# torn8to/sift-based-OD

Hardware: NVIDIA B200
Metric: query descriptors/sec (kNN2+ratio+Hough+affine), 1M-desc DB (higher is better)
Workload: dtype u8

## Files before the change

include/sod.h:

```cpp
#ifndef SOD_H_
#define SOD_H_

#include <stddef.h>
#include <stdint.h>

#ifdef __cplusplus
extern "C" {
#endif

#define SOD_OK 0
#define SOD_ERR_INVALID_ARGUMENT (-1)
#define SOD_ERR_CUDA (-2)
#define SOD_ERR_UNSUPPORTED (-3)

#define SOD_DESC_DIM 128
#define SOD_TILE_ROWS 128
#define SOD_CQ_TILE_INTS 260

typedef void* sod_stream_t;

int sod_version(void);
const char* sod_last_error(void);
int sod_device_sm_count(void);

#define SOD_STAGE_MATCH 0
#define SOD_STAGE_HOUGH_PREP 1
#define SOD_STAGE_HOUGH_VOTE 2
#define SOD_STAGE_HOUGH_FINISH 3
#define SOD_STAGE_AFFINE 4
#define SOD_STAGE_COUNT 5
int sod_timing_enable(int32_t on);
int32_t sod_timing_read(int32_t stage, float* ms_host, int32_t cap);

int64_t sod_cq_ints(int64_t n_rows);

int sod_pack_u8_from_f32(const float* src, int64_t n_rows, uint8_t* dst, int32_t* nonint_flag,
                         sod_stream_t stream);

size_t sod_db_prepare_workspace_bytes(int64_t n_rows);
int sod_db_prepare(const uint8_t* db, int64_t n_rows, uint8_t* db_sorted, int32_t* cq, void* workspace,
                   size_t workspace_bytes, sod_stream_t stream);

int sod_query_prepare(const uint8_t* q, int64_t n_rows, int32_t* qn, sod_stream_t stream);

size_t sod_match_workspace_bytes(int64_t n_query, int64_t n_db);

int sod_match_top2(const uint8_t* q, const int32_t* qn, int64_t n_query, const uint8_t* db_sorted,
                   const int32_t* cq, int64_t n_db, int32_t db_index_base, int32_t* out_idx,
                   uint32_t* out_d2, void* workspace, size_t workspace_bytes, sod_stream_t stream);

int64_t sod_row_thr_ints(int64_t n_query);
int sod_match_top2_range(const uint8_t* q, const int32_t* qn, int64_t n_query, const uint8_t* db_sorted,
                         const int32_t* cq, int64_t n_db, int32_t db_index_base, int64_t tile_begin,
                         int64_t tile_end, int32_t* row_thr, int32_t* out_idx, uint32_t* out_d2,
                         void* workspace, size_t workspace_bytes, sod_stream_t stream);

int sod_match_top2_peer(const uint8_t* q, const int32_t* qn, int64_t n_query, const uint8_t* db_sorted,
                        const int32_t* cq, int64_t n_db, int32_t db_index_base, int64_t tile_begin,
                        int64_t tile_end, int32_t* row_thr, int32_t* const* peer_thr_host, int32_t n_peers,
                        int64_t block_rotation, int32_t* out_idx, uint32_t* out_d2, void* workspace,
                        size_t workspace_bytes, sod_stream_t stream);

int sod_top2_merge(const int32_t* parts_idx, const uint32_t* parts_d2, int32_t n_parts,
                   int64_t n_query, int32_t* out_idx, uint32_t* out_d2, float* out_dist,
                   uint8_t* out_pass, double ratio, sod_stream_t stream);

int sod_top2_keys(const int32_t* idx, const uint32_t* d2, int64_t n_query, int64_t n_rows, int64_t* keys,
                  sod_stream_t stream);
int sod_top2_merge_keys(const int64_t* parts, int32_t n_parts, int64_t n_rows, int64_t* out, sod_stream_t stream);
int sod_top2_from_keys(const int64_t* keys, int64_t n_query, int32_t* out_idx, uint32_t* out_d2, float* out_dist,
                       uint8_t* out_pass, double ratio, sod_stream_t stream);

#define SOD_EXCHANGE_MAX_RANKS 16
#define SOD_IPC_HANDLE_BYTES 64
size_t sod_exchange_bytes(int64_t max_query, int32_t world);
int sod_exchange_alloc(size_t bytes, void** buffer_out);
int sod_exchange_free(void* buffer);
int sod_ipc_export(const void* buffer, uint8_t* handle_host);
int sod_ipc_open(const uint8_t* handle_host, void** buffer_out);
int sod_ipc_close(void* buffer);
int sod_top2_exchange_peer(const int32_t* idx, const uint32_t* d2, int64_t n_query, int32_t rank, int32_t world,
                           void* const* peer_buffers_host, int64_t max_query, int32_t* out_idx, uint32_t* out_d2,
                           float* out_dist, uint8_t* out_pass, double ratio, sod_stream_t stream);


int64_t sod_bf16_operand_cols(int32_t split);
int64_t sod_bf16_db_rows(int64_t n_rows);

int sod_bf16_prepare(const float* src, int64_t n_rows, int32_t side, int32_t split, uint16_t* dst,
                     float* norms, int32_t* nonfinite_flag, sod_stream_t stream);

size_t sod_match_bf16_workspace_bytes(int64_t n_query, int64_t n_db);

int sod_match_top2_bf16(const uint16_t* q_op, const float* qn, int64_t n_query, const uint16_t* db_op,
                        const float* dn, int64_t n_db, int32_t split, int32_t db_index_base,
                        int32_t* out_idx, float* out_d2, void* workspace, size_t workspace_bytes,
                        sod_stream_t stream);

int sod_top2_merge_f32(const int32_t* parts_idx, const float* parts_d2, int32_t n_parts,
                       int64_t n_query, int32_t* out_idx, float* out_d2, float* out_dist,
                       uint8_t* out_pass, double ratio, sod_stream_t stream);



typedef struct {
  const float* xy;
  const float* angle;
  const int32_t* octave;
  int64_t n;
} sod_keypoints;

typedef struct {
  sod_keypoints query;
  const int32_t* query_frame;
  const int32_t* frame_wh;
  int32_t n_frames;
  sod_keypoints model;
  const int32_t* model_image;
  const double* image_centroid;
  const double* image_size;
  const int32_t* image_group;
  int32_t n_images;
  int32_t groups_per_frame;
} sod_scene;

#define SOD_SIGMA_LUT_MIN (-24)
#define SOD_SIGMA_LUT_LEN 49
#define SOD_MAX_BINS 15
#define SOD_MAX_CLUSTER_BINS 65536

typedef struct {
  double* pose;
  uint32_t* base_bin;
  uint8_t* near_edge;
  int32_t* counters;
  int32_t* bin_group;
  int32_t* bin_code;
  int32_t* bin_count;
  int32_t* bin_offset;
  int64_t* bin_order;
  double* bin_mean;
  int32_t* members;
  int64_t cap_bins;
  int64_t cap_votes;
} sod_hough_out;

size_t sod_compact_scratch_bytes(int64_t n_query);
int sod_compact_matches(const int32_t* idx, const uint8_t* pass, int64_t n_query, int32_t t_lo,
                        int32_t t_hi, int32_t* match_q, int32_t* match_t, int32_t* n_out,
                        void* scratch, sod_stream_t stream);

int sod_estimate_pose(const sod_scene* scene, const int32_t* match_q, const int32_t* match_t,
                      int64_t n_matches, int32_t bins, const int32_t* sigma_lut, double* pose,
                      uint32_t* base_bin, uint8_t* near_edge, sod_stream_t stream);

int sod_pose_bin_index(const double* pose, int64_t n, int32_t bins, int32_t width, int32_t height,
                       const int32_t* sigma_lut, uint32_t* base_bin, sod_stream_t stream);

size_t sod_hough_workspace_bytes(int64_t n_matches, int64_t n_groups);

int sod_hough_vote(const sod_scene* scene, const int32_t* match_q, const int32_t* match_t,
                   int64_t n_matches, const int32_t* n_matches_dev, int32_t bins,
                   const int32_t* sigma_lut, int32_t detail_min_count, const sod_hough_out* out,
                   void* workspace, size_t workspace_bytes, sod_stream_t stream);

int sod_hough_vote_dims(const sod_scene* scene, const int32_t* match_q, const int32_t* match_t,
                        int64_t n_matches, const int32_t* n_matches_dev, int32_t bins_x, int32_t bins_y,
                        int32_t bins_theta, int32_t bins_sigma, const int32_t* sigma_lut,
                        int32_t detail_min_count, const sod_hough_out* out, void* workspace,
                        size_t workspace_bytes, sod_stream_t stream);

typedef struct {
  int32_t* counters;
  int32_t* valid_bin;
  double* params;
  int32_t* votes;
  int32_t* status;
  uint8_t* member_keep;
  int64_t cap_valid;
  int64_t cap_votes;
} sod_affine_out;

int sod_affine_verify(const sod_scene* scene, const int32_t* match_q, const int32_t* match_t,
                      const sod_hough_out* hough, int32_t bins, int32_t vote_threshold,
                      int32_t affine_threshold, double factor_x, double factor_y, int32_t max_passes,
                      const sod_affine_out* out, sod_stream_t stream);

int sod_valid_bin_records(const sod_hough_out* hough, const sod_affine_out* affine, int32_t* out_group,
                          int32_t* out_code, int64_t* out_order, double* out_mean, sod_stream_t stream);

int sod_affine_residual_keep(const float* model_xy, const float* query_xy, int64_t n,
                             const double* params, double x_ref, double y_ref, uint8_t* keep,
                             sod_stream_t stream);


int sod_pose_adjacency(const double* cx, const double* cy, const double* reach_x, const double* reach_y,
                       const int32_t* segment, int64_t n, uint32_t* adj, int32_t* label,
                       sod_stream_t stream);

int sod_angle_adjacency(const double* angle, const int32_t* segment, int64_t n, double max_degrees,
                        uint32_t* adj, int32_t* label, sod_stream_t stream);


#define SOD_SIFT_MAX_OCTAVES 16
#define SOD_SIFT_MAX_CAP (1 << 24)

typedef struct {
  float* xy;
  float* size;
  float* angle;
  float* response;
  int32_t* octave;
  uint8_t* des;
  int32_t* counters;
  int64_t cap;
} sod_sift_out;

size_t sod_sift_workspace_bytes(int32_t width, int32_t height, int64_t max_keypoints);

int sod_sift_extract(const uint8_t* gray, int32_t width, int32_t height, int64_t pitch, const sod_sift_out* out,
                     void* workspace, size_t workspace_bytes, sod_stream_t stream);

int sod_sift_describe(const uint8_t* gray, int32_t width, int32_t height, int64_t pitch, const float* xy,
                      const float* size, const float* angle, const int32_t* octave, int64_t n, uint8_t* des,
                      int32_t* n_invalid, void* workspace, size_t workspace_bytes, sod_stream_t stream);

int64_t sod_sift_level_offset(int32_t width, int32_t height, int32_t octave, int32_t level, int32_t* wh_host);

#ifdef __cplusplus
}
#endif
#endif
```

sift-based-od_b200/csrc/sod_capi.cu:

```cuda
#include <cstring>

#include "sod_common.cuh"

namespace sod {

namespace {
thread_local char g_err[512] = {0};
}

void set_error(const char* fmt, ...) {
  va_list ap;
  va_start(ap, fmt);
  vsnprintf(g_err, sizeof(g_err), fmt, ap);
  va_end(ap);
}

namespace {
constexpr int kTimerRing = 128;
struct StageTimers {
  bool on = false;
  cudaEvent_t ev[SOD_STAGE_COUNT][kTimerRing][2] = {};
  int head[SOD_STAGE_COUNT] = {};
  bool open[SOD_STAGE_COUNT] = {};
};
thread_local StageTimers g_timers;
}

void stage_begin(int stage, cudaStream_t st) {
  StageTimers& t = g_timers;
  if (!t.on || stage < 0 || stage >= SOD_STAGE_COUNT || t.head[stage] >= kTimerRing) return;
  cudaEvent_t& e = t.ev[stage][t.head[stage]][0];
  if (!e && cudaEventCreate(&e) != cudaSuccess) return;
  t.open[stage] = cudaEventRecord(e, st) == cudaSuccess;
}

void stage_end(int stage, cudaStream_t st) {
  StageTimers& t = g_timers;
  if (!t.on || stage < 0 || stage >= SOD_STAGE_COUNT || !t.open[stage]) return;
  t.open[stage] = false;
  cudaEvent_t& e = t.ev[stage][t.head[stage]][1];
  if (!e && cudaEventCreate(&e) != cudaSuccess) return;
  if (cudaEventRecord(e, st) == cudaSuccess) ++t.head[stage];
}

int device_sm_count() {
  int dev = 0, sms = 0;
  if (cudaGetDevice(&dev) != cudaSuccess ||
      cudaDeviceGetAttribute(&sms, cudaDevAttrMultiProcessorCount, dev) != cudaSuccess) {
    set_error("cannot query the current CUDA device: %s", cudaGetErrorString(cudaGetLastError()));
    return -1;
  }
  return sms;
}

}

extern "C" {

int sod_version(void) { return 2000; }

const char* sod_last_error(void) { return sod::g_err; }

int sod_device_sm_count(void) { return sod::device_sm_count(); }

int sod_timing_enable(int32_t on) {
  sod::g_timers.on = on != 0;
  for (int s = 0; s < SOD_STAGE_COUNT; ++s) {
    sod::g_timers.head[s] = 0;
    sod::g_timers.open[s] = false;
  }
  return SOD_OK;
}

int32_t sod_timing_read(int32_t stage, float* ms_host, int32_t cap) {
  sod::StageTimers& t = sod::g_timers;
  if (stage < 0 || stage >= SOD_STAGE_COUNT || (cap > 0 && !ms_host)) {
    sod::set_error("sod_timing_read: bad stage or null buffer");
    return SOD_ERR_INVALID_ARGUMENT;
  }
  const int n = t.head[stage];
  int out = 0;
  for (int i = 0; i < n; ++i) {
    float ms = 0.f;
    if (cudaEventSynchronize(t.ev[stage][i][1]) != cudaSuccess ||
        cudaEventElapsedTime(&ms, t.ev[stage][i][0], t.ev[stage][i][1]) != cudaSuccess) {
      sod::set_error("sod_timing_read: %s", cudaGetErrorString(cudaGetLastError()));
      t.head[stage] = 0;
      return SOD_ERR_CUDA;
    }
    if (out < cap) ms_host[out++] = ms;
  }
  t.head[stage] = 0;
  return out;
}

}
```

sift-based-od_b200/csrc/sod_match.cu:

```cuda
#include <climits>
#include <cub/device/device_radix_sort.cuh>

#include "sod_common.cuh"
#include "sod_ptx.cuh"
#include "sod_tma.cuh"
#include "sod_top2.cuh"

namespace sod {
namespace {

constexpr int kTileM = 128;
constexpr int kQTiles = 4;
constexpr int kBlockQ = kTileM * kQTiles;
constexpr int kAbiBlockQ = 256;
constexpr int kTileN = SOD_TILE_ROWS;
constexpr int kTileBytes = kTileN * SOD_DESC_DIM;
constexpr int kChunk = 32;
constexpr int kCqTile = SOD_CQ_TILE_INTS;
constexpr int kCqPerm = kTileN + 4;
constexpr int kCqTileBytes = kCqTile * 4;
constexpr int kNoKey = 0x7FFFFF;
constexpr int kEpiWarps = 4 * kQTiles;
constexpr int kIssuers = 2;
constexpr int kThreads = (4 + kEpiWarps) * 32;
constexpr int kTmemCols = 512;
constexpr int kRegsLight = 56;
constexpr int kRegsEpilogue = 104;
constexpr int kRegsLaunch = 65536 / kThreads / 8 * 8;
static_assert(128 * kRegsLight + kEpiWarps * 32 * kRegsEpilogue <= kThreads * kRegsLaunch,
              "setmaxnreg budget exceeds the CTA's register pool");

static_assert(kQTiles * kTileN == kTmemCols, "one 128-column accumulator slot per query tile fills TMEM");

constexpr int kStages = 8;
constexpr int kBStageBytes = kTileBytes / 2;
constexpr int kCqSlots = 16;
constexpr int kOffA = 0;
constexpr int kOffB = kOffA + 2 * kQTiles * kTileBytes;
constexpr int kOffCq = kOffB + kStages * kBStageBytes;
constexpr int kOffBar = kOffCq + kCqSlots * kCqTileBytes;
constexpr int kNumBars = 2 * kStages + 4 + 2 * kQTiles + kCqSlots;
constexpr int kOffTmemPtr = kOffBar + kNumBars * 8;
constexpr int kSmemBytes = kOffTmemPtr + 16 + 1024;
static_assert(kCqSlots >= kStages + 2 && (kCqSlots & (kCqSlots - 1)) == 0, "cq ring too shallow");
static_assert(kSmemBytes <= 227 * 1024, "shared memory exceeds the 227 KB a block may use");

struct MatchArgs {
  const int32_t* qn;
  const int32_t* cq;
  uint32_t* part_d2;
  int32_t* part_idx;
  int32_t* row_thr;
  int nq;
  int thr_rows;
  int n_tiles;
  int tile_begin;
  int n_qunits;
  int n_seg;
  int idx_base;
  int n_peers;
  int unit_rot;
  int32_t* peer_thr[SOD_EXCHANGE_MAX_RANKS];
};

__device__ __forceinline__ int imax3(int a, int b, int c) { return max(max(a, b), c); }
struct Top2 {
  long long k1, k2;
  int d2;
  __device__ __forceinline__ void offer(int d, int i) {
    const long long key = (static_cast<long long>(d) << 32) | static_cast<unsigned>(i);
    if (key < k1) {
      k2 = k1;
      k1 = key;
    } else if (key < k2) {
      k2 = key;
    }
    d2 = static_cast<int>(k2 >> 32);
  }
};
constexpr long long kNoKey64 = (static_cast<long long>(kNoKey) << 32) | 0x7FFFFFFF;

__device__ __forceinline__ void top2_chunk(const uint32_t* v, const int4* __restrict__ cp4,
                                           int cmin, const int32_t* __restrict__ perm_s,
                                           int idx_base, Top2& best, int& thr) {
  const int* av = reinterpret_cast<const int*>(v);
  int t[11];
#pragma unroll
  for (int i = 0; i < 10; ++i) t[i] = imax3(av[3 * i], av[3 * i + 1], av[3 * i + 2]);
  t[10] = max(av[30], av[31]);
  const int u0 = imax3(t[0], t[1], t[2]), u1 = imax3(t[3], t[4], t[5]), u2 = imax3(t[6], t[7], t[8]);
  const int u3 = max(t[9], t[10]);
  if (cmin - 2 * max(imax3(u0, u1, u2), u3) > thr) return;
  const int* cp = reinterpret_cast<const int*>(cp4);
  int t1 = INT_MAX, t2 = INT_MAX;
  auto scan = [&](int lo, int hi) {
#pragma unroll
    for (int j = lo; j < hi; ++j) {
      const int key = cp[j] - 512 * av[j];
      const int m = max(t1, key);
      t1 = min(t1, key);
      t2 = min(t2, m);
    }
  };
  if (cmin - 2 * u0 <= thr) scan(0, 9);
  if (cmin - 2 * u1 <= thr) scan(9, 18);
  if (cmin - 2 * u2 <= thr) scan(18, 27);
  if (cmin - 2 * u3 <= thr) scan(27, 32);
  if ((t1 >> 8) > thr) return;
  SOD_DCHECK((t1 & 0xFF) < kTileN && (t2 == INT_MAX || (t2 & 0xFF) < kTileN));
  const int o1 = perm_s[t1 & 0xFF];
  if (o1 >= 0) best.offer(t1 >> 8, idx_base + o1);
  thr = min(thr, best.d2);
  if ((t2 >> 8) <= thr) {
    const int o2 = perm_s[t2 & 0xFF];
    if (o2 >= 0) best.offer(t2 >> 8, idx_base + o2);
    thr = min(thr, best.d2);
  }
}

template <bool kShare, bool kSeeded = false>
__global__ void __launch_bounds__(kThreads, 1)
match_top2_kernel(const __grid_constant__ CUtensorMap tmap_q,
                  const __grid_constant__ CUtensorMap tmap_db, const MatchArgs a) {
  extern __shared__ uint8_t smem_raw[];
  const uint32_t raw_addr = smem_u32(smem_raw);
  const uint32_t base = (raw_addr + 1023u) & ~1023u;
  uint8_t* smem = smem_raw + (base - raw_addr);

  const int warp = threadIdx.x >> 5;
  const int lane = threadIdx.x & 31;
  const uint32_t cta_rank = cluster_ctarank();
  const int unit0 = static_cast<int>(cluster_id_x());
  const int unit_step = static_cast<int>(cluster_count_x());

  const uint32_t bar0 = base + kOffBar;
  auto bar_full = [&](int s) { return bar0 + 8u * s; };
  auto bar_empty = [&](int s) { return bar0 + 8u * (kStages + s); };
  auto bar_afull = [&](int b) { return bar0 + 8u * (2 * kStages + b); };
  auto bar_aempty = [&](int b) { return bar0 + 8u * (2 * kStages + 2 + b); };
  auto bar_tfull = [&](int h) { return bar0 + 8u * (2 * kStages + 4 + h); };
  auto bar_tempty = [&](int h) { return bar0 + 8u * (2 * kStages + 4 + kQTiles + h); };
  auto bar_cqfull = [&](int s) { return bar0 + 8u * (2 * kStages + 4 + 2 * kQTiles + s); };
  volatile uint32_t* tmem_ptr_smem = reinterpret_cast<volatile uint32_t*>(smem + kOffTmemPtr);

  if (warp == 0 && lane == 0) {
    tma_prefetch_desc(&tmap_q);
    tma_prefetch_desc(&tmap_db);
  }
  if (warp == 1 && lane == 0) {
    for (int s = 0; s < kStages; ++s) {
      mbar_init(bar_full(s), 1);
      mbar_init(bar_empty(s), kIssuers);
    }
    for (int b = 0; b < 2; ++b) {
      mbar_init(bar_afull(b), 1);
      mbar_init(bar_aempty(b), kIssuers);
    }
    for (int h = 0; h < kQTiles; ++h) {
      mbar_init(bar_tfull(h), 1);
      mbar_init(bar_tempty(h), 8);
    }
    for (int s = 0; s < kCqSlots; ++s) mbar_init(bar_cqfull(s), 1);
    fence_mbar_init();
  }
  if (warp == 2) {
    tmem_alloc_pair(smem_u32(const_cast<uint32_t*>(tmem_ptr_smem)), kTmemCols);
    tmem_relinquish_pair();
  }
  tc_fence_before();
  cluster_sync_all();
  tc_fence_after();
  const uint32_t tmem_base = *tmem_ptr_smem;

  const int total_units = a.n_qunits * a.n_seg;

  if (warp < 4) {
    if constexpr (kRegsLight < kRegsLaunch)
      setmaxnreg_dec<kRegsLight>();
  if (warp == 0) {
    if (lane == 0) {
      uint32_t step = 0, ucount = 0;
      for (int u = unit0; u < total_units; u += unit_step, ++ucount) {
        const int seg = u / a.n_qunits;
        int qu = u - seg * a.n_qunits + a.unit_rot;
        if (qu >= a.n_qunits) qu -= a.n_qunits;
        const int qb = qu * 2 + static_cast<int>(cta_rank);
        const int t0 = a.tile_begin + static_cast<int>(static_cast<int64_t>(seg) * a.n_tiles / a.n_seg);
        const int t1 = a.tile_begin + static_cast<int>(static_cast<int64_t>(seg + 1) * a.n_tiles / a.n_seg);
        const uint32_t ab = ucount & 1u, aph = (ucount >> 1) & 1u;
        mbar_wait(bar_aempty(ab), aph ^ 1u);
        if (cta_rank == 0) mbar_arrive_expect_tx(bar_afull(ab), 2 * kQTiles * kTileBytes);
        const uint32_t afull_leader = mapa_shared(bar_afull(ab), 0);
        for (int h = 0; h < kQTiles; ++h)
          tma_load_2d_pair(base + kOffA + (ab * kQTiles + h) * kTileBytes, &tmap_q, afull_leader, 0,
                           qb * kBlockQ + h * kTileM);
        for (int t = t0; t < t1; ++t, ++step) {
          const uint32_t s = step % kStages, ph = (step / kStages) & 1u;
          mbar_wait(bar_empty(s), ph ^ 1u);
          if (cta_rank == 0) mbar_arrive_expect_tx(bar_full(s), 2 * kBStageBytes);
          tma_load_2d_pair(base + kOffB + s * kBStageBytes, &tmap_db, mapa_shared(bar_full(s), 0), 0,
                           t * kTileN + static_cast<int>(cta_rank) * (kTileN / 2));
          const uint32_t slot = step % kCqSlots;
          mbar_arrive_expect_tx(bar_cqfull(slot), kCqTileBytes);
          bulk_load_1d(base + kOffCq + slot * kCqTileBytes, a.cq + static_cast<int64_t>(t) * kCqTile,
                       kCqTileBytes, bar_cqfull(slot));
        }
      }
    }
  } else if ((warp == 1 || warp == 3) && cta_rank == 0) {
    const int h0 = warp >> 1;
    constexpr uint32_t idesc = umma_idesc_u8(2 * kTileM, kTileN);
    uint32_t step = 0, ucount = 0;
    for (int u = unit0; u < total_units; u += unit_step, ++ucount) {
      const int seg = u / a.n_qunits;
      const int t0 = a.tile_begin + static_cast<int>(static_cast<int64_t>(seg) * a.n_tiles / a.n_seg);
      const int t1 = a.tile_begin + static_cast<int>(static_cast<int64_t>(seg + 1) * a.n_tiles / a.n_seg);
      const uint32_t ab = ucount & 1u, aph = (ucount >> 1) & 1u;
      mbar_wait(bar_afull(ab), aph);
      const uint32_t a_buf = base + kOffA + ab * (kQTiles * kTileBytes);
      for (int t = t0; t < t1; ++t, ++step) {
        const uint32_t s = step % kStages, ph = (step / kStages) & 1u;
        const uint64_t bdesc = umma_desc_k128(base + kOffB + s * kBStageBytes);
        mbar_wait(bar_full(s), ph);
#pragma unroll
        for (int i = 0; i < kQTiles / kIssuers; ++i) {
          const int h = h0 + kIssuers * i;
          const uint64_t adesc = umma_desc_k128(a_buf + h * kTileBytes);
          if (step >= 1)
            mbar_wait(bar_tempty(h), (step - 1) & 1u);
          tc_fence_after();
          if (elect_one()) {
#pragma unroll
            for (int k = 0; k < SOD_DESC_DIM / 32; ++k)
              umma_i8_pair(tmem_base + h * kTileN, adesc + 2 * k, bdesc + 2 * k, idesc, k > 0);
            umma_commit_pair(bar_tfull(h), 3);
            if (i == kQTiles / kIssuers - 1) umma_commit_pair(bar_empty(s), 3);
          }
          __syncwarp();
        }
      }
      if (elect_one()) umma_commit_pair(bar_aempty(ab), 3);
      __syncwarp();
    }
  }
  } else {
    if constexpr (kRegsEpilogue > kRegsLaunch) setmaxnreg_inc<kRegsEpilogue>();
    const int e = warp - 4;
    const int quad = warp & 3;
    const int h = e >> 2;
    const uint32_t lane_sel = static_cast<uint32_t>(quad * 32) << 16;
    uint32_t tfull_h = bar_tfull(h);
    uint32_t cqfull_0 = bar_cqfull(0);
    uint32_t cq_0 = base + kOffCq;
    uint32_t taddr = tmem_base + lane_sel + h * kTileN;
    asm volatile("" : "+r"(tfull_h), "+r"(cqfull_0), "+r"(taddr), "+r"(cq_0));
    uint32_t tempty_rel = mapa_shared(bar_tempty(h), 0);
    asm volatile("" : "+r"(tempty_rel));
    uint32_t step = 0, ucount = 1;
    for (int u = unit0; u < total_units; u += unit_step, ++ucount) {
      const int seg = u / a.n_qunits;
      int qu = u - seg * a.n_qunits + a.unit_rot;
      if (qu >= a.n_qunits) qu -= a.n_qunits;
      const int qb = qu * 2 + static_cast<int>(cta_rank);
      const int t0 = a.tile_begin + static_cast<int>(static_cast<int64_t>(seg) * a.n_tiles / a.n_seg);
      const int t1 = a.tile_begin + static_cast<int>(static_cast<int64_t>(seg + 1) * a.n_tiles / a.n_seg);
      const int row = qb * kBlockQ + h * kTileM + quad * 32 + lane;
      Top2 best{kNoKey64, kNoKey64, kNoKey};
      const bool thr_row = (kShare || kSeeded) && row < a.thr_rows;
      int* const gthr = (kShare || kSeeded) ? a.row_thr + row : nullptr;
      int published = kNoKey;
      int thr = thr_row ? min(kNoKey, __ldcg(gthr)) : kNoKey;
      const uint32_t step_end = step + static_cast<uint32_t>(t1 - t0);
      for (; step < step_end; ++step) {
        const uint32_t slot = step % kCqSlots, cqph = (step / kCqSlots) & 1u;
        mbar_wait(cqfull_0 + 8u * slot, cqph);
        mbar_wait(tfull_h, step & 1u);
        tc_fence_after();
        const int32_t* cs = reinterpret_cast<const int32_t*>(__cvta_shared_to_generic(cq_0 + slot * kCqTileBytes));
        const int32_t* perm_s = cs + kCqPerm;
        const int g_next = (kShare && thr_row) ? __ldcg(gthr) : kNoKey;
        const int4* c4 = reinterpret_cast<const int4*>(cs);
        const int4 cmin = c4[kTileN / 4];
        uint32_t v[2 * kChunk];
        tmem_ld64_wait(taddr, v);
        top2_chunk(v, c4, cmin.x, perm_s, a.idx_base, best, thr);
        top2_chunk(v + kChunk, c4 + 8, cmin.y, perm_s, a.idx_base, best, thr);
        tmem_ld64_wait(taddr + 2 * kChunk, v);
        tc_fence_before();
        __syncwarp();
        if (lane == 0) mbar_arrive_cluster(tempty_rel);
        top2_chunk(v, c4 + 16, cmin.z, perm_s, a.idx_base, best, thr);
        top2_chunk(v + kChunk, c4 + 24, cmin.w, perm_s, a.idx_base, best, thr);
        if (kShare && thr_row) {
          if (best.d2 < published) {
            published = best.d2;
            atomicMin(gthr, published);
          }
          thr = min(thr, g_next);
        }
      }
      if (kSeeded && thr_row && best.d2 < kNoKey) {
        if (a.n_peers > 0) {
          const int64_t slot = gthr - a.row_thr;
          for (int p = 0; p < a.n_peers; ++p) atomicMin(a.peer_thr[p] + slot, best.d2);
        } else {
          atomicMin(gthr, best.d2);
        }
      }
      if (row < a.nq) {
        const int qn = a.qn[row];
        const int64_t o = (static_cast<int64_t>(seg) * a.nq + row) * 2;
        SOD_DCHECK(seg < a.n_seg && (best.k1 == kNoKey64 || static_cast<int>(best.k1 & 0xFFFFFFFFll) >= a.idx_base));
        const int d1 = static_cast<int>(best.k1 >> 32), d2 = static_cast<int>(best.k2 >> 32);
        a.part_d2[o + 0] = d1 != kNoKey ? static_cast<uint32_t>(d1 + qn) : 0xFFFFFFFFu;
        a.part_d2[o + 1] = d2 != kNoKey ? static_cast<uint32_t>(d2 + qn) : 0xFFFFFFFFu;
        a.part_idx[o + 0] = d1 != kNoKey ? static_cast<int>(best.k1 & 0xFFFFFFFFll) : -1;
        a.part_idx[o + 1] = d2 != kNoKey ? static_cast<int>(best.k2 & 0xFFFFFFFFll) : -1;
      }
    }
  }

  tc_fence_before();
  cluster_sync_all();
  if (warp == 2) tmem_dealloc_pair(tmem_base, kTmemCols);
}

__global__ void row_sqnorm_kernel(const uint8_t* __restrict__ x, int64_t n_rows,
                                  int32_t* __restrict__ out) {
  const int64_t t = static_cast<int64_t>(blockIdx.x) * blockDim.x + threadIdx.x;
  const int64_t row = t >> 3;
  const int part = threadIdx.x & 7;
  uint32_t s = 0;
  if (row < n_rows) {
    const uint4 w = __ldg(reinterpret_cast<const uint4*>(x + row * SOD_DESC_DIM) + part);
    s = __dp4a(w.x, w.x, s);
    s = __dp4a(w.y, w.y, s);
    s = __dp4a(w.z, w.z, s);
    s = __dp4a(w.w, w.w, s);
  }
#pragma unroll
  for (int o = 4; o > 0; o >>= 1) s += __shfl_xor_sync(0xffffffffu, s, o);
  if (part == 0 && row < n_rows) out[row] = static_cast<int32_t>(s);
}

__global__ void db_norm_kernel(const uint8_t* __restrict__ db, int64_t n_rows,
                               uint32_t* __restrict__ keys, int32_t* __restrict__ vals) {
  const int64_t row = static_cast<int64_t>(blockIdx.x) * blockDim.x + threadIdx.x;
  if (row >= n_rows) return;
  const uint4* p = reinterpret_cast<const uint4*>(db + row * SOD_DESC_DIM);
  uint32_t s = 0;
#pragma unroll
  for (int j = 0; j < SOD_DESC_DIM / 16; ++j) {
    const uint4 w = __ldg(p + j);
    s = __dp4a(w.x, w.x, s);
    s = __dp4a(w.y, w.y, s);
    s = __dp4a(w.z, w.z, s);
    s = __dp4a(w.w, w.w, s);
  }
  keys[row] = s;
  vals[row] = static_cast<int32_t>(row);
}

__global__ void __launch_bounds__(kTileN)
db_tile_kernel(const uint8_t* __restrict__ db, int64_t n_rows, int64_t n_tiles, int64_t stride,
               const uint32_t* __restrict__ keys, const int32_t* __restrict__ vals,
               uint8_t* __restrict__ db_sorted, int32_t* __restrict__ cq) {
  __shared__ int s_idx[kTileN];
  __shared__ int s_c[kTileN];
  const int64_t tile = blockIdx.x;
  const int64_t rank = (tile * stride) % n_tiles;
  const int col = threadIdx.x;
  const int64_t src_pos = rank * kTileN + col;
  const int64_t pos = tile * kTileN + col;
  s_idx[col] = src_pos < n_rows ? vals[src_pos] : INT_MAX;
  s_c[col] = src_pos < n_rows ? static_cast<int>(keys[src_pos]) : kNoKey;
  __syncthreads();
  for (int k = 2; k <= kTileN; k <<= 1) {
    for (int j = k >> 1; j > 0; j >>= 1) {
      const int partner = col ^ j;
      if (partner > col) {
        const bool up = (col & k) == 0;
        const int a = s_idx[col], b = s_idx[partner];
        if ((a > b) == up) {
          s_idx[col] = b; s_idx[partner] = a;
          const int ca = s_c[col];
          s_c[col] = s_c[partner]; s_c[partner] = ca;
        }
      }
      __syncthreads();
    }
  }
  const int idx = s_idx[col];
  const int c = s_c[col];
  int32_t* out = cq + tile * kCqTile;
  out[col] = (c << 8) | col;
  out[kCqPerm + col] = idx == INT_MAX ? -1 : idx;
  int cm = c;
#pragma unroll
  for (int o = 16; o > 0; o >>= 1) cm = min(cm, __shfl_xor_sync(0xffffffffu, cm, o));
  if ((col & 31) == 0) out[kTileN + (col >> 5)] = cm;
  uint4* dst = reinterpret_cast<uint4*>(db_sorted + pos * SOD_DESC_DIM);
  if (idx != INT_MAX) {
    const uint4* src = reinterpret_cast<const uint4*>(db + static_cast<int64_t>(idx) * SOD_DESC_DIM);
#pragma unroll
    for (int j = 0; j < SOD_DESC_DIM / 16; ++j) dst[j] = __ldg(src + j);
  } else {
#pragma unroll
    for (int j = 0; j < SOD_DESC_DIM / 16; ++j) dst[j] = make_uint4(0, 0, 0, 0);
  }
}

struct PrepWs {
  uint32_t *keys_in, *keys_out;
  int32_t *vals_in, *vals_out;
  void* cub_temp;
  size_t cub_bytes, bytes;
};

PrepWs carve_prep_ws(void* base, int64_t n) {
  PrepWs w;
  size_t o = 0;
  auto take = [&](size_t bytes) {
    void* p = base ? static_cast<char*>(base) + o : nullptr;
    o += (bytes + 255) & ~static_cast<size_t>(255);
    return p;
  };
  w.keys_in = static_cast<uint32_t*>(take(n * 4));
  w.keys_out = static_cast<uint32_t*>(take(n * 4));
  w.vals_in = static_cast<int32_t*>(take(n * 4));
  w.vals_out = static_cast<int32_t*>(take(n * 4));
  w.cub_bytes = 0;
  cub::DeviceRadixSort::SortPairs(nullptr, w.cub_bytes, w.keys_in, w.keys_out, w.vals_in, w.vals_out,
                                  static_cast<int>(n), 0, 24);
  w.cub_temp = take(w.cub_bytes);
  w.bytes = o;
  return w;
}

__global__ void pack_u8_kernel(const float4* __restrict__ src, int64_t n_vec4,
                               uchar4* __restrict__ dst, int32_t* __restrict__ nonint_flag) {
  const int64_t i = static_cast<int64_t>(blockIdx.x) * blockDim.x + threadIdx.x;
  if (i >= n_vec4) return;
  const float4 f = src[i];
  const float r[4] = {f.x, f.y, f.z, f.w};
  unsigned char b[4];
  bool bad = false;
#pragma unroll
  for (int k = 0; k < 4; ++k) {
    const float c = fminf(fmaxf(r[k], 0.f), 255.f);
    const float q = rintf(c);
    bad |= !(q == r[k]);
    b[k] = static_cast<unsigned char>(q);
  }
  dst[i] = make_uchar4(b[0], b[1], b[2], b[3]);
  if (bad) atomicOr(nonint_flag, 1);
}

__global__ void top2_merge_kernel(const int32_t* __restrict__ parts_idx,
                                  const uint32_t* __restrict__ parts_d2, int n_parts, int64_t nq,
                                  int32_t* __restrict__ out_idx, uint32_t* __restrict__ out_d2,
                                  float* __restrict__ out_dist, uint8_t* __restrict__ out_pass,
                                  double ratio) {
  const int64_t row = static_cast<int64_t>(blockIdx.x) * blockDim.x + threadIdx.x;
  if (row >= nq) return;
  uint32_t d1 = 0xFFFFFFFFu, d2 = 0xFFFFFFFFu;
  int32_t i1 = -1, i2 = -1;
  for (int p = 0; p < n_parts; ++p) {
    const int64_t o = (static_cast<int64_t>(p) * nq + row) * 2;
    const int2 ci = *reinterpret_cast<const int2*>(parts_idx + o);
    const uint2 cd = *reinterpret_cast<const uint2*>(parts_d2 + o);
#pragma unroll
    for (int j = 0; j < 2; ++j) {
      const int32_t ci_j = j ? ci.y : ci.x;
      const uint32_t cd_j = j ? cd.y : cd.x;
      if (ci_j < 0) continue;
      const bool lt1 = i1 < 0 || cd_j < d1 || (cd_j == d1 && ci_j < i1);
      const bool lt2 = i2 < 0 || cd_j < d2 || (cd_j == d2 && ci_j < i2);
      if (lt1) {
        d2 = d1; i2 = i1;
        d1 = cd_j; i1 = ci_j;
      } else if (lt2) {
        d2 = cd_j; i2 = ci_j;
      }
    }
  }
  write_top2_row(row, i1, d1, i2, d2, out_idx, out_d2, out_dist, out_pass, ratio);
}

__global__ void top2_keys_kernel(const int32_t* __restrict__ idx, const uint32_t* __restrict__ d2, int64_t nq,
                                 int64_t n_rows, longlong2* __restrict__ keys) {
  const int64_t row = static_cast<int64_t>(blockIdx.x) * blockDim.x + threadIdx.x;
  if (row >= n_rows) return;
  longlong2 k = make_longlong2(kNoneKey, kNoneKey);
  if (row < nq)
    k = top2_pack_keys(*reinterpret_cast<const int2*>(idx + row * 2), *reinterpret_cast<const uint2*>(d2 + row * 2));
  keys[row] = k;
}

__global__ void top2_merge_keys_kernel(const longlong2* __restrict__ parts, int n_parts, int64_t n_rows,
                                       longlong2* __restrict__ out) {
  const int64_t row = static_cast<int64_t>(blockIdx.x) * blockDim.x + threadIdx.x;
  if (row >= n_rows) return;
  long long k1 = kNoneKey, k2 = kNoneKey;
  for (int p = 0; p < n_parts; ++p) top2_fold_keys(k1, k2, parts[static_cast<int64_t>(p) * n_rows + row]);
  out[row] = make_longlong2(k1, k2);
}

__global__ void top2_from_keys_kernel(const longlong2* __restrict__ keys, int64_t nq,
                                      int32_t* __restrict__ out_idx, uint32_t* __restrict__ out_d2,
                                      float* __restrict__ out_dist, uint8_t* __restrict__ out_pass, double ratio) {
  const int64_t row = static_cast<int64_t>(blockIdx.x) * blockDim.x + threadIdx.x;
  if (row >= nq) return;
  const longlong2 k = keys[row];
  write_top2_keys_row(row, k.x, k.y, out_idx, out_d2, out_dist, out_pass, ratio);
}

struct Plan {
  int n_tiles, n_qblocks, n_qunits, n_seg, grid;
};

constexpr int kUnitFillSteps = 6;

Plan make_plan(int64_t nq, int64_t ndb, int sms) {
  Plan p;
  p.n_tiles = static_cast<int>((ndb + kTileN - 1) / kTileN);
  p.n_qblocks = static_cast<int>((nq + kBlockQ - 1) / kBlockQ);
  p.n_qunits = (p.n_qblocks + 1) / 2;
  const int pairs = sms / 2;
  p.n_seg = 1;
  if (p.n_tiles > 0 && p.n_qblocks > 0) {
    const int max_seg = p.n_tiles < 512 ? p.n_tiles : 512;
    int64_t best = -1;
    for (int s = 1; s <= max_seg; ++s) {
      const int64_t units = static_cast<int64_t>(p.n_qunits) * s;
      const int64_t waves = (units + pairs - 1) / pairs;
      const int64_t cost = waves * ((p.n_tiles + s - 1) / s + kUnitFillSteps);
      if (best < 0 || cost < best) {
        best = cost;
        p.n_seg = s;
      }
    }
  }
  const int64_t units = static_cast<int64_t>(p.n_qunits) * p.n_seg;
  p.grid = static_cast<int>(units < pairs ? units : pairs) * 2;
  return p;
}

int make_desc_map(CUtensorMap* m, const uint8_t* ptr, int64_t n_rows, int box_rows = kTileN) {
  return make_rowmajor_map(m, CU_TENSOR_MAP_DATA_TYPE_UINT8, 1, ptr, n_rows, SOD_DESC_DIM, SOD_DESC_DIM,
                           box_rows);
}

}
}

using namespace sod;

extern "C" {

int64_t sod_cq_ints(int64_t n_rows) {
  return n_rows <= 0 ? 0 : (n_rows + kTileN - 1) / kTileN * kCqTile;
}

int sod_pack_u8_from_f32(const float* src, int64_t n_rows, uint8_t* dst, int32_t* nonint_flag,
                         sod_stream_t stream) {
  SOD_CHECK_ARG(n_rows >= 0, "n_rows < 0");
  if (n_rows == 0) return SOD_OK;
  SOD_CHECK_ARG(src && dst && nonint_flag, "null pointer");
  const int64_t n4 = n_rows * (SOD_DESC_DIM / 4);
  const int threads = 256;
  pack_u8_kernel<<<static_cast<unsigned>((n4 + threads - 1) / threads), threads, 0,
                   static_cast<cudaStream_t>(stream)>>>(reinterpret_cast<const float4*>(src), n4,
                                                        reinterpret_cast<uchar4*>(dst), nonint_flag);
  SOD_CHECK_LAUNCH("pack_u8_kernel");
  return SOD_OK;
}

size_t sod_db_prepare_workspace_bytes(int64_t n_rows) {
  if (n_rows <= 0) return 256;
  return carve_prep_ws(nullptr, n_rows).bytes + 256;
}

int sod_db_prepare(const uint8_t* db, int64_t n_rows, uint8_t* db_sorted, int32_t* cq, void* workspace,
                   size_t workspace_bytes, sod_stream_t stream) {
  SOD_CHECK_ARG(n_rows >= 0 && n_rows < (int64_t(1) << 31) - kTileN, "n_rows out of range");
  if (n_rows == 0) return SOD_OK;
  SOD_CHECK_ARG(db && db_sorted && cq && workspace, "null pointer");
  SOD_CHECK_ARG(db != db_sorted, "db_sorted must not alias db");
  SOD_CHECK_ARG((reinterpret_cast<uintptr_t>(db) & 15) == 0 && (reinterpret_cast<uintptr_t>(db_sorted) & 15) == 0 &&
                    (reinterpret_cast<uintptr_t>(workspace) & 255) == 0,
                "db/db_sorted must be 16-byte and workspace 256-byte aligned");
  PrepWs w = carve_prep_ws(workspace, n_rows);
  SOD_CHECK_ARG(workspace_bytes >= w.bytes, "workspace too small: %zu < %zu", workspace_bytes, w.bytes);
  cudaStream_t st = static_cast<cudaStream_t>(stream);
  const int threads = 128;
  db_norm_kernel<<<static_cast<unsigned>((n_rows + threads - 1) / threads), threads, 0, st>>>(
      db, n_rows, w.keys_in, w.vals_in);
  SOD_CHECK_LAUNCH("db_norm_kernel");
  SOD_CHECK_CUDA(cub::DeviceRadixSort::SortPairs(w.cub_temp, w.cub_bytes, w.keys_in, w.keys_out, w.vals_in,
                                                 w.vals_out, static_cast<int>(n_rows), 0, 24, st));
  const int64_t tiles = (n_rows + kTileN - 1) / kTileN;
  int64_t stride = static_cast<int64_t>(0.6180339887498949 * static_cast<double>(tiles)) | 1;
  auto gcd = [](int64_t a, int64_t b) { while (b) { const int64_t t = a % b; a = b; b = t; } return a; };
  while (gcd(stride, tiles) != 1) stride += 2;
  db_tile_kernel<<<static_cast<unsigned>(tiles), kTileN, 0, st>>>(db, n_rows, tiles, stride, w.keys_out,
                                                                 w.vals_out, db_sorted, cq);
  SOD_CHECK_LAUNCH("db_tile_kernel");
  return SOD_OK;
}

int sod_query_prepare(const uint8_t* q, int64_t n_rows, int32_t* qn, sod_stream_t stream) {
  SOD_CHECK_ARG(n_rows >= 0 && n_rows < (int64_t(1) << 31) - kBlockQ, "n_rows out of range");
  if (n_rows == 0) return SOD_OK;
  SOD_CHECK_ARG(q && qn, "null pointer");
  const int threads = 256;
  const int64_t blocks = (n_rows * 8 + threads - 1) / threads;
  row_sqnorm_kernel<<<static_cast<unsigned>(blocks), threads, 0, static_cast<cudaStream_t>(stream)>>>(
      q, n_rows, qn);
  SOD_CHECK_LAUNCH("row_sqnorm_kernel");
  return SOD_OK;
}

static int64_t thr_rows(int64_t n_query) {
  return n_query <= 0 ? 0 : (n_query + kAbiBlockQ - 1) / kAbiBlockQ * kAbiBlockQ;
}
static size_t match_lists_bytes(const Plan& p, int64_t n_query) {
  return static_cast<size_t>(p.n_seg) * static_cast<size_t>(n_query) * 2 * 8;
}
static size_t match_workspace_need(const Plan& p, int64_t n_query) {
  return match_lists_bytes(p, n_query) + static_cast<size_t>(thr_rows(n_query)) * 4;
}

int64_t sod_row_thr_ints(int64_t n_query) { return thr_rows(n_query); }

size_t sod_match_workspace_bytes(int64_t n_query, int64_t n_db) {
  if (n_query <= 0 || n_db <= 0) return 16;
  const int sms = device_sm_count();
  return match_workspace_need(make_plan(n_query, n_db, sms >= 2 ? sms : 148), n_query) + 16;
}

int sod_match_top2(const uint8_t* q, const int32_t* qn, int64_t n_query, const uint8_t* db_sorted,
                   const int32_t* cq, int64_t n_db, int32_t db_index_base, int32_t* out_idx,
                   uint32_t* out_d2, void* workspace, size_t workspace_bytes, sod_stream_t stream) {
  return sod_match_top2_range(q, qn, n_query, db_sorted, cq, n_db, db_index_base, 0, -1, nullptr, out_idx, out_d2,
                              workspace, workspace_bytes, stream);
}

int sod_match_top2_range(const uint8_t* q, const int32_t* qn, int64_t n_query, const uint8_t* db_sorted,
                         const int32_t* cq, int64_t n_db, int32_t db_index_base, int64_t tile_begin,
                         int64_t tile_end, int32_t* row_thr, int32_t* out_idx, uint32_t* out_d2,
                         void* workspace, size_t workspace_bytes, sod_stream_t stream) {
  return sod_match_top2_peer(q, qn, n_query, db_sorted, cq, n_db, db_index_base, tile_begin, tile_end, row_thr, nullptr, 0,
                             0, out_idx, out_d2, workspace, workspace_bytes, stream);
}

int sod_match_top2_peer(const uint8_t* q, const int32_t* qn, int64_t n_query, const uint8_t* db_sorted,
                        const int32_t* cq, int64_t n_db, int32_t db_index_base, int64_t tile_begin,
                        int64_t tile_end, int32_t* row_thr, int32_t* const* peer_thr_host, int32_t n_peers,
                        int64_t block_rotation, int32_t* out_idx, uint32_t* out_d2, void* workspace,
                        size_t workspace_bytes, sod_stream_t stream) {
  SOD_CHECK_ARG(n_peers >= 0 && n_peers <= SOD_EXCHANGE_MAX_RANKS && (n_peers == 0 || (peer_thr_host && row_thr)),
                "bad peer threshold table");
  SOD_CHECK_ARG(block_rotation >= 0, "negative block rotation");
  SOD_CHECK_ARG(n_query >= 0 && n_db >= 0, "negative size");
  SOD_CHECK_ARG(n_query < (int64_t(1) << 31) - 2 * kBlockQ && n_db < (int64_t(1) << 31) - kTileN,
                "size out of range");
  SOD_CHECK_ARG(static_cast<int64_t>(db_index_base) + n_db < (int64_t(1) << 31),
                "db_index_base + n_db overflows int32");
  if (n_query == 0) return SOD_OK;
  SOD_CHECK_ARG(out_idx && out_d2, "null output pointer");
  cudaStream_t st = static_cast<cudaStream_t>(stream);
  const int mthreads = 128;
  const unsigned mblocks = static_cast<unsigned>((n_query + mthreads - 1) / mthreads);
  const int64_t all_tiles = (n_db + kTileN - 1) / kTileN;
  if (tile_end < 0) tile_end = all_tiles;
  SOD_CHECK_ARG(tile_begin >= 0 && tile_begin <= tile_end && tile_end <= all_tiles, "tile range out of bounds");
  if (n_db == 0 || tile_begin == tile_end) {
    top2_merge_kernel<<<mblocks, mthreads, 0, st>>>(nullptr, nullptr, 0, n_query, out_idx, out_d2,
                                                    nullptr, nullptr, 0.0);
    SOD_CHECK_LAUNCH("top2_merge_kernel");
    return SOD_OK;
  }
  const uint8_t* db = db_sorted;
  SOD_CHECK_ARG(q && qn && db && cq && workspace, "null pointer");
  SOD_CHECK_ARG((reinterpret_cast<uintptr_t>(q) & 15) == 0 && (reinterpret_cast<uintptr_t>(db) & 15) == 0 &&
                    (reinterpret_cast<uintptr_t>(cq) & 15) == 0 &&
                    (reinterpret_cast<uintptr_t>(workspace) & 15) == 0,
                "q, db, cq and workspace must be 16-byte aligned");
  const int sms = device_sm_count();
  if (sms <= 0) return SOD_ERR_CUDA;
  if (sms < 2) {
    set_error("sod_match_top2: the matcher runs on CTA pairs and needs at least 2 SMs, the device has %d", sms);
    return SOD_ERR_UNSUPPORTED;
  }
  const Plan p = make_plan(n_query, (tile_end - tile_begin) * kTileN, sms);
  const size_t need = match_workspace_need(p, n_query);
  SOD_CHECK_ARG(workspace_bytes >= need, "workspace too small: %zu < %zu", workspace_bytes, need);

  CUtensorMap map_q, map_db;
  int rc = make_desc_map(&map_q, q, n_query);
  if (rc != SOD_OK) return rc;
  rc = make_desc_map(&map_db, db, (n_db + kTileN - 1) / kTileN * kTileN, kTileN / 2);
  if (rc != SOD_OK) return rc;

  MatchArgs a;
  a.qn = qn;
  a.cq = cq;
  a.part_d2 = static_cast<uint32_t*>(workspace);
  a.part_idx = reinterpret_cast<int32_t*>(a.part_d2 + static_cast<size_t>(p.n_seg) * n_query * 2);
  a.row_thr = row_thr;
  if (!row_thr && p.n_seg > 1) {
    a.row_thr = reinterpret_cast<int32_t*>(static_cast<uint8_t*>(workspace) + match_lists_bytes(p, n_query));
    SOD_CHECK_CUDA(cudaMemsetAsync(a.row_thr, 0x7F, static_cast<size_t>(thr_rows(n_query)) * 4, st));
  }
  a.nq = static_cast<int>(n_query);
  a.thr_rows = static_cast<int>(thr_rows(n_query));
  a.n_tiles = p.n_tiles;
  a.tile_begin = static_cast<int>(tile_begin);
  a.n_qunits = p.n_qunits;
  a.n_seg = p.n_seg;
  a.idx_base = db_index_base;
  const bool peer_mode = n_peers > 0 && row_thr && p.n_seg == 1;
  a.n_peers = peer_mode ? n_peers : 0;
  a.unit_rot = peer_mode ? static_cast<int>((block_rotation / (2 * kBlockQ / kAbiBlockQ)) % p.n_qunits) : 0;
  for (int i = 0; i < SOD_EXCHANGE_MAX_RANKS; ++i) a.peer_thr[i] = (peer_mode && i < n_peers) ? peer_thr_host[i] : nullptr;
  for (int i = 0; i < a.n_peers; ++i) SOD_CHECK_ARG(a.peer_thr[i], "null threshold array of rank %d", i);

  const bool seeded = row_thr && p.n_seg == 1, share = a.row_thr && !seeded;
  auto* kernel = seeded ? match_top2_kernel<false, true>
                        : share ? match_top2_kernel<true, false> : match_top2_kernel<false, false>;
  SOD_CHECK_CUDA(cudaFuncSetAttribute(kernel, cudaFuncAttributeMaxDynamicSharedMemorySize, kSmemBytes));
  {
    StageScope timed(SOD_STAGE_MATCH, st);
    cudaLaunchConfig_t cfg = {};
    cfg.gridDim = dim3(static_cast<unsigned>(p.grid));
    cfg.blockDim = dim3(kThreads);
    cfg.dynamicSmemBytes = static_cast<size_t>(kSmemBytes);
    cfg.stream = st;
    cudaLaunchAttribute attr[1];
    attr[0].id = cudaLaunchAttributeClusterDimension;
    attr[0].val.clusterDim.x = 2;
    attr[0].val.clusterDim.y = 1;
    attr[0].val.clusterDim.z = 1;
    cfg.attrs = attr;
    cfg.numAttrs = 1;
    SOD_CHECK_CUDA(cudaLaunchKernelEx(&cfg, kernel, map_q, map_db, a));
  }
  SOD_CHECK_LAUNCH("match_top2_kernel");
  top2_merge_kernel<<<mblocks, mthreads, 0, st>>>(a.part_idx, a.part_d2, p.n_seg, n_query,
                                                  out_idx, out_d2, nullptr, nullptr, 0.0);
  SOD_CHECK_LAUNCH("top2_merge_kernel");
  return SOD_OK;
}

int sod_top2_merge(const int32_t* parts_idx, const uint32_t* parts_d2, int32_t n_parts,
                   int64_t n_query, int32_t* out_idx, uint32_t* out_d2, float* out_dist,
                   uint8_t* out_pass, double ratio, sod_stream_t stream) {
  SOD_CHECK_ARG(n_parts >= 0 && n_query >= 0, "negative size");
  if (n_query == 0) return SOD_OK;
  SOD_CHECK_ARG(out_idx && out_d2, "null output pointer");
  SOD_CHECK_ARG(n_parts == 0 || (parts_idx && parts_d2), "null parts pointer");
  const int threads = 128;
  top2_merge_kernel<<<static_cast<unsigned>((n_query + threads - 1) / threads), threads, 0,
                      static_cast<cudaStream_t>(stream)>>>(parts_idx, parts_d2, n_parts, n_query,
                                                           out_idx, out_d2, out_dist, out_pass, ratio);
  SOD_CHECK_LAUNCH("top2_merge_kernel");
  return SOD_OK;
}

int sod_top2_keys(const int32_t* idx, const uint32_t* d2, int64_t n_query, int64_t n_rows, int64_t* keys,
                  sod_stream_t stream) {
  SOD_CHECK_ARG(n_query >= 0 && n_rows >= n_query, "need 0 <= n_query <= n_rows");
  if (n_rows == 0) return SOD_OK;
  SOD_CHECK_ARG(keys && (n_query == 0 || (idx && d2)), "null pointer");
  SOD_CHECK_ARG((reinterpret_cast<uintptr_t>(keys) & 15) == 0, "keys must be 16-byte aligned");
  const int threads = 256;
  top2_keys_kernel<<<static_cast<unsigned>((n_rows + threads - 1) / threads), threads, 0,
                     static_cast<cudaStream_t>(stream)>>>(idx, d2, n_query, n_rows,
                                                          reinterpret_cast<longlong2*>(keys));
  SOD_CHECK_LAUNCH("top2_keys_kernel");
  return SOD_OK;
}

int sod_top2_merge_keys(const int64_t* parts, int32_t n_parts, int64_t n_rows, int64_t* out, sod_stream_t stream) {
  SOD_CHECK_ARG(n_parts >= 0 && n_rows >= 0, "negative size");
  if (n_rows == 0) return SOD_OK;
  SOD_CHECK_ARG(out && (n_parts == 0 || parts), "null pointer");
  SOD_CHECK_ARG((reinterpret_cast<uintptr_t>(parts) & 15) == 0 && (reinterpret_cast<uintptr_t>(out) & 15) == 0,
                "key arrays must be 16-byte aligned");
  const int threads = 256;
  top2_merge_keys_kernel<<<static_cast<unsigned>((n_rows + threads - 1) / threads), threads, 0,
                           static_cast<cudaStream_t>(stream)>>>(reinterpret_cast<const longlong2*>(parts), n_parts,
                                                                n_rows, reinterpret_cast<longlong2*>(out));
  SOD_CHECK_LAUNCH("top2_merge_keys_kernel");
  return SOD_OK;
}

int sod_top2_from_keys(const int64_t* keys, int64_t n_query, int32_t* out_idx, uint32_t* out_d2, float* out_dist,
                       uint8_t* out_pass, double ratio, sod_stream_t stream) {
  SOD_CHECK_ARG(n_query >= 0, "negative size");
  if (n_query == 0) return SOD_OK;
  SOD_CHECK_ARG(keys && out_idx && out_d2, "null pointer");
  SOD_CHECK_ARG((reinterpret_cast<uintptr_t>(keys) & 15) == 0, "keys must be 16-byte aligned");
  const int threads = 256;
  top2_from_keys_kernel<<<static_cast<unsigned>((n_query + threads - 1) / threads), threads, 0,
                          static_cast<cudaStream_t>(stream)>>>(reinterpret_cast<const longlong2*>(keys), n_query,
                                                               out_idx, out_d2, out_dist, out_pass, ratio);
  SOD_CHECK_LAUNCH("top2_from_keys_kernel");
  return SOD_OK;
}

}
```

sift-based-od_b200/sod_b200/_capi.py:

```python
from __future__ import annotations

import ctypes as C
import os
from pathlib import Path

_LIB_PATH = Path(os.environ.get("SOD_B200_LIB") or Path(__file__).resolve().parent / "libsod_b200.so")

SOD_OK = 0
DESC_DIM = 128
TILE_ROWS = 128


class SodError(RuntimeError):
    pass


def _load() -> C.CDLL:
    if not _LIB_PATH.exists():
        raise ImportError(
            f"{_LIB_PATH} not built: run `python __graft_entry__.py` (or sod_b200.build.build()); "
            "the CUDA library is the only implementation of the hot path")
    return C.CDLL(str(_LIB_PATH))


lib = _load()

_p = C.c_void_p
_i64 = C.c_int64
_i32 = C.c_int32



class Keypoints(C.Structure):
    _fields_ = [("xy", _p), ("angle", _p), ("octave", _p), ("n", _i64)]


class Scene(C.Structure):
    _fields_ = [("query", Keypoints), ("query_frame", _p), ("frame_wh", _p), ("n_frames", _i32),
                ("model", Keypoints), ("model_image", _p), ("image_centroid", _p), ("image_size", _p),
                ("image_group", _p), ("n_images", _i32), ("groups_per_frame", _i32)]


class HoughOut(C.Structure):
    _fields_ = [("pose", _p), ("base_bin", _p), ("near_edge", _p), ("counters", _p), ("bin_group", _p),
                ("bin_code", _p), ("bin_count", _p), ("bin_offset", _p), ("bin_order", _p),
                ("bin_mean", _p), ("members", _p), ("cap_bins", _i64), ("cap_votes", _i64)]


class AffineOut(C.Structure):
    _fields_ = [("counters", _p), ("valid_bin", _p), ("params", _p), ("votes", _p), ("status", _p),
                ("member_keep", _p), ("cap_valid", _i64), ("cap_votes", _i64)]


class SiftOut(C.Structure):
    _fields_ = [("xy", _p), ("size", _p), ("angle", _p), ("response", _p), ("octave", _p), ("des", _p),
                ("counters", _p), ("cap", _i64)]


STAGES = {"match": 0, "hough_prep": 1, "hough_vote": 2, "hough_finish": 3, "affine": 4}


def timing_enable(on: bool = True) -> None:
    check(lib.sod_timing_enable(int(on)), "sod_timing_enable")


def timing_read(stage: str) -> list[float]:
    buf = (C.c_float * 128)()
    n = int(lib.sod_timing_read(STAGES[stage], C.cast(buf, _p), 128))
    if n < 0:
        check(n, "sod_timing_read")
    return [float(buf[i]) for i in range(n)]


SIGMA_LUT_MIN = -24
SIGMA_LUT_LEN = 49
MAX_BINS = 15

_PROTOS = {
    "sod_version": (C.c_int, []),
    "sod_last_error": (C.c_char_p, []),
    "sod_device_sm_count": (C.c_int, []),
    "sod_timing_enable": (C.c_int, [_i32]),
    "sod_timing_read": (_i32, [_i32, _p, _i32]),
    "sod_cq_ints": (_i64, [_i64]),
    "sod_pack_u8_from_f32": (C.c_int, [_p, _i64, _p, _p, _p]),
    "sod_db_prepare_workspace_bytes": (C.c_size_t, [_i64]),
    "sod_db_prepare": (C.c_int, [_p, _i64, _p, _p, _p, C.c_size_t, _p]),
    "sod_query_prepare": (C.c_int, [_p, _i64, _p, _p]),
    "sod_match_workspace_bytes": (C.c_size_t, [_i64, _i64]),
    "sod_match_top2": (C.c_int, [_p, _p, _i64, _p, _p, _i64, _i32, _p, _p, _p, C.c_size_t, _p]),
    "sod_row_thr_ints": (_i64, [_i64]),
    "sod_match_top2_range": (C.c_int, [_p, _p, _i64, _p, _p, _i64, _i32, _i64, _i64, _p, _p, _p, _p, C.c_size_t, _p]),
    "sod_match_top2_peer": (C.c_int, [_p, _p, _i64, _p, _p, _i64, _i32, _i64, _i64, _p, _p, _i32, _i64, _p, _p, _p,
                                      C.c_size_t, _p]),
    "sod_top2_merge": (C.c_int, [_p, _p, _i32, _i64, _p, _p, _p, _p, C.c_double, _p]),
    "sod_top2_keys": (C.c_int, [_p, _p, _i64, _i64, _p, _p]),
    "sod_top2_merge_keys": (C.c_int, [_p, _i32, _i64, _p, _p]),
    "sod_top2_from_keys": (C.c_int, [_p, _i64, _p, _p, _p, _p, C.c_double, _p]),
    "sod_exchange_bytes": (C.c_size_t, [_i64, _i32]),
    "sod_exchange_alloc": (C.c_int, [C.c_size_t, C.POINTER(_p)]),
    "sod_exchange_free": (C.c_int, [_p]),
    "sod_ipc_export": (C.c_int, [_p, _p]),
    "sod_ipc_open": (C.c_int, [_p, C.POINTER(_p)]),
    "sod_ipc_close": (C.c_int, [_p]),
    "sod_top2_exchange_peer": (C.c_int, [_p, _p, _i64, _i32, _i32, _p, _i64, _p, _p, _p, _p, C.c_double, _p]),
    "sod_bf16_operand_cols": (_i64, [_i32]),
    "sod_bf16_db_rows": (_i64, [_i64]),
    "sod_bf16_prepare": (C.c_int, [_p, _i64, _i32, _i32, _p, _p, _p, _p]),
    "sod_match_bf16_workspace_bytes": (C.c_size_t, [_i64, _i64]),
    "sod_match_top2_bf16": (C.c_int, [_p, _p, _i64, _p, _p, _i64, _i32, _i32, _p, _p, _p, C.c_size_t, _p]),
    "sod_top2_merge_f32": (C.c_int, [_p, _p, _i32, _i64, _p, _p, _p, _p, C.c_double, _p]),
    "sod_pose_adjacency": (C.c_int, [_p, _p, _p, _p, _p, _i64, _p, _p, _p]),
    "sod_angle_adjacency": (C.c_int, [_p, _p, _i64, C.c_double, _p, _p, _p]),
    "sod_compact_scratch_bytes": (C.c_size_t, [_i64]),
    "sod_compact_matches": (C.c_int, [_p, _p, _i64, _i32, _i32, _p, _p, _p, _p, _p]),
    "sod_estimate_pose": (C.c_int, [C.POINTER(Scene), _p, _p, _i64, _i32, _p, _p, _p, _p, _p]),
    "sod_pose_bin_index": (C.c_int, [_p, _i64, _i32, _i32, _i32, _p, _p, _p]),
    "sod_affine_residual_keep": (C.c_int, [_p, _p, _i64, _p, C.c_double, C.c_double, _p, _p]),
    "sod_hough_workspace_bytes": (C.c_size_t, [_i64, _i64]),
    "sod_hough_vote": (C.c_int, [C.POINTER(Scene), _p, _p, _i64, _p, _i32, _p, _i32, C.POINTER(HoughOut), _p,
                                 C.c_size_t, _p]),
    "sod_hough_vote_dims": (C.c_int, [C.POINTER(Scene), _p, _p, _i64, _p, _i32, _i32, _i32, _i32, _p, _i32,
                                      C.POINTER(HoughOut), _p, C.c_size_t, _p]),
    "sod_valid_bin_records": (C.c_int, [C.POINTER(HoughOut), C.POINTER(AffineOut), _p, _p, _p, _p, _p]),
    "sod_affine_verify": (C.c_int, [C.POINTER(Scene), _p, _p, C.POINTER(HoughOut), _i32, _i32, _i32,
                                    C.c_double, C.c_double, _i32, C.POINTER(AffineOut), _p]),
    "sod_sift_workspace_bytes": (C.c_size_t, [_i32, _i32, _i64]),
    "sod_sift_extract": (C.c_int, [_p, _i32, _i32, _i64, C.POINTER(SiftOut), _p, C.c_size_t, _p]),
    "sod_sift_describe": (C.c_int, [_p, _i32, _i32, _i64, _p, _p, _p, _p, _i64, _p, _p, _p, C.c_size_t, _p]),
    "sod_sift_level_offset": (_i64, [_i32, _i32, _i32, _i32, _p]),
}


def _bind() -> None:
    for name, (res, args) in _PROTOS.items():
        fn = getattr(lib, name)
        fn.restype = res
        fn.argtypes = args


_bind()

EXPORTED = tuple(_PROTOS)


def check(rc: int, what: str) -> None:
    if rc != SOD_OK:
        msg = lib.sod_last_error().decode("utf-8", "replace")
        raise SodError(f"{what} failed ({rc}): {msg}")
```

sift-based-od_b200/sod_b200/engine.py:

```python
from __future__ import annotations

import ctypes as C
from dataclasses import dataclass

import numpy as np
import torch

from . import _capi
from ._capi import check, lib

RATIO = 0.75


def _stream() -> C.c_void_p:
    return C.c_void_p(torch.cuda.current_stream().cuda_stream)


def _ptr(t: torch.Tensor | None) -> C.c_void_p:
    return C.c_void_p(0 if t is None else t.data_ptr())


def _require_cuda(t: torch.Tensor, dtype: torch.dtype, name: str) -> torch.Tensor:
    if not t.is_cuda:
        raise ValueError(f"{name} must live on the GPU (no CPU path exists)")
    if t.dtype != dtype:
        raise TypeError(f"{name} must be {dtype}, got {t.dtype}")
    return t.contiguous()


def pack_descriptors(des, device: torch.device | str = "cuda") -> torch.Tensor:
    t = torch.as_tensor(des)
    if t.ndim != 2 or t.shape[1] != _capi.DESC_DIM:
        raise ValueError(f"descriptors must be [n,{_capi.DESC_DIM}], got {tuple(t.shape)}")
    if t.dtype == torch.uint8:
        return t.to(device, non_blocking=True).contiguous()
    if t.dtype != torch.float32:
        raise TypeError(f"descriptors must be float32 or uint8, got {t.dtype}")
    src = t.to(device, non_blocking=True).contiguous()
    dst = torch.empty(src.shape, dtype=torch.uint8, device=src.device)
    flag = torch.zeros(1, dtype=torch.int32, device=src.device)
    check(lib.sod_pack_u8_from_f32(_ptr(src), src.shape[0], _ptr(dst), _ptr(flag), _stream()),
          "sod_pack_u8_from_f32")
    if int(flag.item()) != 0:
        raise NonIntegerDescriptors("descriptors are not integer-valued in 0..255: the exact u8 tensor-core "
                                    "path does not apply (use prepare_db_float / FloatMatcher)")
    return dst


class NonIntegerDescriptors(ValueError):
    """Raised by pack_descriptors for float descriptors the exact u8 path cannot represent."""


@dataclass
class DescriptorShard:
    des: torch.Tensor
    n_rows: int
    cq: torch.Tensor
    index_base: int

    @property
    def n(self) -> int:
        return self.n_rows


def prepare_db(des_u8: torch.Tensor, index_base: int = 0) -> DescriptorShard:
    des_u8 = _require_cuda(des_u8, torch.uint8, "database descriptors")
    n = int(des_u8.shape[0])
    dev = des_u8.device
    tiles = (n + _capi.TILE_ROWS - 1) // _capi.TILE_ROWS
    cq = torch.empty(max(int(lib.sod_cq_ints(n)), 1), dtype=torch.int32, device=dev)
    des_sorted = torch.empty((max(tiles * _capi.TILE_ROWS, 1), _capi.DESC_DIM), dtype=torch.uint8, device=dev)
    ws = torch.empty(int(lib.sod_db_prepare_workspace_bytes(n)), dtype=torch.uint8, device=dev)
    check(lib.sod_db_prepare(_ptr(des_u8), n, _ptr(des_sorted), _ptr(cq), _ptr(ws), ws.numel(),
                             _stream()), "sod_db_prepare")
    return DescriptorShard(des_sorted, n, cq, int(index_base))


class Matcher:

    def __init__(self, shard: DescriptorShard):
        self.shard = shard
        self._ws: torch.Tensor | None = None
        self._qn: torch.Tensor | None = None
        self.events: list | None = None

    @property
    def n_tiles(self) -> int:
        return (self.shard.n + _capi.TILE_ROWS - 1) // _capi.TILE_ROWS

    def new_thresholds(self, nq: int) -> torch.Tensor:
        return torch.full((max(int(lib.sod_row_thr_ints(nq)), 1),), 0x7F7F7F7F, dtype=torch.int32,
                          device=self.shard.des.device)

    def _scratch(self, nq: int, rows: int | None = None) -> tuple[torch.Tensor, torch.Tensor]:
        need = int(lib.sod_match_workspace_bytes(nq, self.shard.n if rows is None else rows))
        dev = self.shard.des.device
        if self._ws is None or self._ws.numel() < need:
            self._ws = torch.empty(need, dtype=torch.uint8, device=dev)
        if self._qn is None or self._qn.numel() < nq:
            self._qn = torch.empty(max(nq, 1), dtype=torch.int32, device=dev)
        return self._ws, self._qn

    def top2(self, q_u8: torch.Tensor, tiles: tuple[int, int] | None = None, row_thr: torch.Tensor | None = None,
             prepared: bool = False, peer_table=None, block_rotation: int = 0) -> tuple[torch.Tensor, torch.Tensor]:
        q_u8 = _require_cuda(q_u8, torch.uint8, "query descriptors")
        nq = int(q_u8.shape[0])
        t0, t1 = (0, self.n_tiles) if tiles is None else (int(tiles[0]), int(tiles[1]))
        ws, qn = self._scratch(nq, (t1 - t0) * _capi.TILE_ROWS)
        idx = torch.empty((nq, 2), dtype=torch.int32, device=q_u8.device)
        d2 = torch.empty((nq, 2), dtype=torch.int32, device=q_u8.device)
        s = self.shard
        if not prepared:
            check(lib.sod_query_prepare(_ptr(q_u8), nq, _ptr(qn), _stream()), "sod_query_prepare")
        if self.events is not None:
            e0, e1 = torch.cuda.Event(enable_timing=True), torch.cuda.Event(enable_timing=True)
            e0.record()
        n_peers = 0 if peer_table is None else len(peer_table)
        check(lib.sod_match_top2_peer(_ptr(q_u8), _ptr(qn), nq, _ptr(s.des), _ptr(s.cq), s.n, s.index_base, t0, t1,
                                      _ptr(row_thr), None if peer_table is None else C.cast(peer_table, C.c_void_p),
                                      n_peers, int(block_rotation), _ptr(idx), _ptr(d2), _ptr(ws), ws.numel(),
                                      _stream()), "sod_match_top2_peer")
        if self.events is not None:
            e1.record()
            self.events.append((e0, e1))
        return idx, d2


def merge_top2(parts_idx: torch.Tensor, parts_d2: torch.Tensor, ratio: float = RATIO):
    parts_idx = _require_cuda(parts_idx, torch.int32, "parts_idx")
    parts_d2 = _require_cuda(parts_d2, torch.int32, "parts_d2")
    if parts_idx.ndim == 2:
        parts_idx, parts_d2 = parts_idx[None], parts_d2[None]
    g, nq = int(parts_idx.shape[0]), int(parts_idx.shape[1])
    dev = parts_idx.device
    idx = torch.empty((nq, 2), dtype=torch.int32, device=dev)
    d2 = torch.empty((nq, 2), dtype=torch.int32, device=dev)
    dist = torch.empty((nq, 2), dtype=torch.float32, device=dev)
    ok = torch.empty(nq, dtype=torch.uint8, device=dev)
    check(lib.sod_top2_merge(_ptr(parts_idx), _ptr(parts_d2), g, nq, _ptr(idx), _ptr(d2), _ptr(dist),
                             _ptr(ok), float(ratio), _stream()), "sod_top2_merge")
    return idx, d2, dist, ok


def top2_keys(idx: torch.Tensor, d2: torch.Tensor, n_rows: int | None = None) -> torch.Tensor:
    idx = _require_cuda(idx, torch.int32, "idx")
    d2 = _require_cuda(d2, torch.int32, "d2")
    nq = int(idx.shape[0])
    n_rows = nq if n_rows is None else int(n_rows)
    keys = torch.empty((n_rows, 2), dtype=torch.int64, device=idx.device)
    check(lib.sod_top2_keys(_ptr(idx), _ptr(d2), nq, n_rows, _ptr(keys), _stream()), "sod_top2_keys")
    return keys


def merge_keys(parts: torch.Tensor) -> torch.Tensor:
    parts = _require_cuda(parts, torch.int64, "parts")
    g, rows = int(parts.shape[0]), int(parts.shape[1])
    out = torch.empty((rows, 2), dtype=torch.int64, device=parts.device)
    check(lib.sod_top2_merge_keys(_ptr(parts), g, rows, _ptr(out), _stream()), "sod_top2_merge_keys")
    return out


def top2_from_keys(keys: torch.Tensor, nq: int, ratio: float = RATIO):
    keys = _require_cuda(keys, torch.int64, "keys")
    dev = keys.device
    idx = torch.empty((nq, 2), dtype=torch.int32, device=dev)
    d2 = torch.empty((nq, 2), dtype=torch.int32, device=dev)
    dist = torch.empty((nq, 2), dtype=torch.float32, device=dev)
    ok = torch.empty(nq, dtype=torch.uint8, device=dev)
    check(lib.sod_top2_from_keys(_ptr(keys), nq, _ptr(idx), _ptr(d2), _ptr(dist), _ptr(ok), float(ratio),
                                 _stream()), "sod_top2_from_keys")
    return idx, d2, dist, ok


def exchange_merge_top2(idx: torch.Tensor, d2: torch.Tensor, world: int, all_to_all, all_gather,
                        ratio: float = RATIO):
    nq = int(idx.shape[0])
    per = (nq + world - 1) // world
    keys = top2_keys(idx, d2, per * world)
    parts = torch.empty_like(keys)
    all_to_all(parts, keys)
    mine = merge_keys(parts.view(world, per, 2))
    merged = torch.empty_like(keys)
    all_gather(merged, mine)
    return top2_from_keys(merged, nq, ratio)


def knn_match_ratio(q_u8: torch.Tensor, matcher: Matcher, ratio: float = RATIO):
    idx, d2 = matcher.top2(q_u8)
    return merge_top2(idx[None], d2[None], ratio)


@dataclass
class FloatShard:
    op: torch.Tensor
    norms: torch.Tensor
    n_rows: int
    index_base: int
    split: bool

    @property
    def n(self) -> int:
        return self.n_rows


def _bf16_prepare(des_f32: torch.Tensor, side: int, split: bool):
    des_f32 = _require_cuda(des_f32, torch.float32, "float descriptors")
    n = int(des_f32.shape[0])
    dev = des_f32.device
    cols = int(lib.sod_bf16_operand_cols(int(split)))
    rows = int(lib.sod_bf16_db_rows(n)) if side else n
    op = torch.empty((max(rows, 1), cols), dtype=torch.int16, device=dev)
    norms = torch.empty(max(rows, 1), dtype=torch.float32, device=dev)
    flag = torch.zeros(1, dtype=torch.int32, device=dev)
    check(lib.sod_bf16_prepare(_ptr(des_f32), n, side, int(split), _ptr(op), _ptr(norms), _ptr(flag), _stream()),
          "sod_bf16_prepare")
    if int(flag.item()) != 0:
        raise ValueError("descriptors contain NaN or infinite values")
    return op, norms


def prepare_db_float(des_f32: torch.Tensor, index_base: int = 0, split: bool = True) -> FloatShard:
    op, norms = _bf16_prepare(des_f32, 1, split)
    return FloatShard(op, norms, int(des_f32.shape[0]), int(index_base), bool(split))


class FloatMatcher:

    def __init__(self, shard: FloatShard):
        self.shard = shard
        self._ws: torch.Tensor | None = None
        self.events: list | None = None

    def top2(self, q_f32: torch.Tensor) -> tuple[torch.Tensor, torch.Tensor]:
        s = self.shard
        q_op, qn = _bf16_prepare(q_f32, 0, s.split)
        nq = int(q_f32.shape[0])
        need = int(lib.sod_match_bf16_workspace_bytes(nq, s.n))
        if self._ws is None or self._ws.numel() < need:
            self._ws = torch.empty(need, dtype=torch.uint8, device=q_op.device)
        idx = torch.empty((nq, 2), dtype=torch.int32, device=q_op.device)
        d2 = torch.empty((nq, 2), dtype=torch.float32, device=q_op.device)
        if self.events is not None:
            e0, e1 = torch.cuda.Event(enable_timing=True), torch.cuda.Event(enable_timing=True)
            e0.record()
        check(lib.sod_match_top2_bf16(_ptr(q_op), _ptr(qn), nq, _ptr(s.op), _ptr(s.norms), s.n, int(s.split),
                                      s.index_base, _ptr(idx), _ptr(d2), _ptr(self._ws), self._ws.numel(),
                                      _stream()), "sod_match_top2_bf16")
        if self.events is not None:
            e1.record()
            self.events.append((e0, e1))
        return idx, d2


def merge_top2_float(parts_idx: torch.Tensor, parts_d2: torch.Tensor, ratio: float = RATIO):
    parts_idx = _require_cuda(parts_idx, torch.int32, "parts_idx")
    parts_d2 = _require_cuda(parts_d2, torch.float32, "parts_d2")
    if parts_idx.ndim == 2:
        parts_idx, parts_d2 = parts_idx[None], parts_d2[None]
    g, nq = int(parts_idx.shape[0]), int(parts_idx.shape[1])
    dev = parts_idx.device
    idx = torch.empty((nq, 2), dtype=torch.int32, device=dev)
    d2 = torch.empty((nq, 2), dtype=torch.float32, device=dev)
    dist = torch.empty((nq, 2), dtype=torch.float32, device=dev)
    ok = torch.empty(nq, dtype=torch.uint8, device=dev)
    check(lib.sod_top2_merge_f32(_ptr(parts_idx), _ptr(parts_d2), g, nq, _ptr(idx), _ptr(d2), _ptr(dist),
                                 _ptr(ok), float(ratio), _stream()), "sod_top2_merge_f32")
    return idx, d2, dist, ok


def knn_match_ratio_float(q_f32: torch.Tensor, matcher: FloatMatcher, ratio: float = RATIO):
    idx, d2 = matcher.top2(q_f32)
    return merge_top2_float(idx[None], d2[None], ratio)


import math

from ._capi import AffineOut, HoughOut, Keypoints, Scene

POS_FACTOR = 32
N_OCT = 4


def sigma_lut(bins: int) -> list[int]:
    out = []
    for k in range(_capi.SIGMA_LUT_MIN, _capi.SIGMA_LUT_MIN + _capi.SIGMA_LUT_LEN):
        i = int(math.log(2.0 ** k, 2) / (2 * (N_OCT - 1) + 0.5) * bins)
        out.append(min(max(0, i), bins - 1))
    return out


def _dev(x, dtype, device):
    t = torch.as_tensor(x)
    return t.to(device=device, dtype=dtype, non_blocking=True).contiguous()


class SceneArrays:

    def __init__(self, q_xy, q_angle, q_octave, m_xy, m_angle, m_octave, m_image, img_centroid, img_size,
                 frame_wh, q_frame=None, img_group=None, groups_per_frame: int = 1, device="cuda"):
        d = torch.device(device)
        self.q_xy = _dev(q_xy, torch.float32, d).reshape(-1, 2)
        self.q_angle = _dev(q_angle, torch.float32, d)
        self.q_octave = _dev(q_octave, torch.int32, d)
        self.m_xy = _dev(m_xy, torch.float32, d).reshape(-1, 2)
        self.m_angle = _dev(m_angle, torch.float32, d)
        self.m_octave = _dev(m_octave, torch.int32, d)
        self.m_image = _dev(m_image, torch.int32, d)
        self.img_centroid = _dev(img_centroid, torch.float64, d).reshape(-1, 2)
        self.img_size = _dev(img_size, torch.float64, d).reshape(-1, 2)
        self.frame_wh = _dev(frame_wh, torch.int32, d).reshape(-1, 2)
        self.q_frame = None if q_frame is None else _dev(q_frame, torch.int32, d)
        self.img_group = None if img_group is None else _dev(img_group, torch.int32, d)
        self.groups_per_frame = int(groups_per_frame)
        self.device = d
        n_img = self.img_centroid.shape[0]
        if self.img_size.shape[0] != n_img or self.m_image.numel() != self.m_xy.shape[0]:
            raise ValueError("inconsistent model arrays")

    @property
    def n_frames(self) -> int:
        return int(self.frame_wh.shape[0])

    @property
    def n_groups(self) -> int:
        return self.n_frames * self.groups_per_frame

    def struct(self) -> Scene:
        return Scene(
            Keypoints(_ptr(self.q_xy), _ptr(self.q_angle), _ptr(self.q_octave), self.q_xy.shape[0]),
            _ptr(self.q_frame), _ptr(self.frame_wh), self.n_frames,
            Keypoints(_ptr(self.m_xy), _ptr(self.m_angle), _ptr(self.m_octave), self.m_xy.shape[0]),
            _ptr(self.m_image), _ptr(self.img_centroid), _ptr(self.img_size), _ptr(self.img_group),
            int(self.img_centroid.shape[0]), self.groups_per_frame)


def compact_matches(idx: torch.Tensor, ok: torch.Tensor, t_lo: int = 0, t_hi: int = 2 ** 31 - 1):
    idx = _require_cuda(idx, torch.int32, "idx")
    ok = _require_cuda(ok, torch.uint8, "pass flags")
    nq = int(ok.shape[0])
    dev = idx.device
    mq = torch.empty(max(nq, 1), dtype=torch.int32, device=dev)
    mt = torch.empty(max(nq, 1), dtype=torch.int32, device=dev)
    n = torch.zeros(1, dtype=torch.int32, device=dev)
    scratch = torch.empty(int(lib.sod_compact_scratch_bytes(nq)), dtype=torch.uint8, device=dev)
    check(lib.sod_compact_matches(_ptr(idx), _ptr(ok), nq, int(t_lo), int(t_hi), _ptr(mq), _ptr(mt), _ptr(n),
                                  _ptr(scratch), _stream()), "sod_compact_matches")
    return mq, mt, n


class HoughResult:

    def __init__(self, m_cap: int, n_groups: int, bins, device):
        self.dims = tuple(bins) if isinstance(bins, (tuple, list)) else (int(bins),) * 4
        self.bins = self.dims[3]
        self.m_cap = m_cap
        nb4 = int(np.prod(self.dims))
        self.cap_bins = max(1, min(16 * m_cap, n_groups * nb4))
        self.cap_votes = max(1, 16 * m_cap)
        e = lambda n, dt: torch.empty(n, dtype=dt, device=device)
        self.pose = e((max(m_cap, 1), 4), torch.float64)
        self.base_bin = e(max(m_cap, 1), torch.int32)
        self.near_edge = e(max(m_cap, 1), torch.uint8)
        self.counters = torch.zeros(8, dtype=torch.int32, device=device)
        self.bin_group = e(self.cap_bins, torch.int32)
        self.bin_code = e(self.cap_bins, torch.int32)
        self.bin_count = e(self.cap_bins, torch.int32)
        self.bin_offset = e(self.cap_bins, torch.int32)
        self.bin_order = e(self.cap_bins, torch.int64)
        self.bin_mean = e((self.cap_bins, 6), torch.float64)
        self.members = e(self.cap_votes, torch.int32)

    def struct(self) -> HoughOut:
        return HoughOut(_ptr(self.pose), _ptr(self.base_bin), _ptr(self.near_edge), _ptr(self.counters),
                        _ptr(self.bin_group), _ptr(self.bin_code), _ptr(self.bin_count),
                        _ptr(self.bin_offset), _ptr(self.bin_order), _ptr(self.bin_mean),
                        _ptr(self.members), self.cap_bins, self.cap_votes)

    def host(self) -> dict:
        c = self.counters.cpu().numpy()
        if c[3]:
            raise _capi.SodError("Hough output capacity exceeded")
        nb, nv = int(c[0]), int(c[1])
        order = torch.argsort(self.bin_order[:nb])
        g = lambda t: t[:nb][order].cpu().numpy()
        return dict(n_bins=nb, n_votes=nv, n_near_edge=int(c[2]), n_unresolved_edge=int(c[4]), rec=order.cpu().numpy(),
                    group=g(self.bin_group), code=g(self.bin_code), count=g(self.bin_count),
                    offset=g(self.bin_offset), mean=g(self.bin_mean), order_key=g(self.bin_order),
                    members=self.members[:nv].cpu().numpy())


class HoughVoter:

    def __init__(self, scene: SceneArrays, bins=15):
        self.dims = tuple(int(b) for b in bins) if isinstance(bins, (tuple, list)) else (int(bins),) * 4
        if len(self.dims) != 4 or min(self.dims) < 1:
            raise ValueError("bins must be a positive int or four positive ints")
        if max(self.dims) > 255 or int(np.prod(self.dims)) > _capi.MAX_BINS ** 4:
            raise _capi.SodError(f"bins={bins}: more than {_capi.MAX_BINS}^4 counters are not supported by the "
                                 f"shared-memory histogram")
        self.scene = scene
        self.bins = self.dims[0] if len(set(self.dims)) == 1 else None
        self.lut = torch.tensor(sigma_lut(self.dims[3]), dtype=torch.int32, device=scene.device)
        self._ws = None
        self._res: HoughResult | None = None

    def reserve(self, m_cap: int) -> HoughResult:
        if self._res is None or self._res.m_cap < int(m_cap):
            self._res = HoughResult(int(m_cap), self.scene.n_groups, self.dims, self.scene.device)
        return self._res

    def new_result(self, m_cap: int) -> HoughResult:
        return HoughResult(int(m_cap), self.scene.n_groups, self.dims, self.scene.device)

    def vote(self, match_q: torch.Tensor, match_t: torch.Tensor, n_dev: torch.Tensor | None = None,
             detail_min_count: int = 1, result: HoughResult | None = None) -> HoughResult:
        match_q = _require_cuda(match_q, torch.int32, "match_q")
        match_t = _require_cuda(match_t, torch.int32, "match_t")
        m = int(match_q.shape[0])
        sc = self.scene
        need = int(lib.sod_hough_workspace_bytes(m, sc.n_groups))
        if self._ws is None or self._ws.numel() < need:
            self._ws = torch.empty(need, dtype=torch.uint8, device=sc.device)
        if result is not None and result.m_cap < m:
            raise ValueError(f"HoughResult sized for {result.m_cap} matches cannot take {m}")
        res = result if result is not None else self.reserve(m)
        s, o = sc.struct(), res.struct()
        check(lib.sod_hough_vote_dims(C.byref(s), _ptr(match_q), _ptr(match_t), m, _ptr(n_dev), *self.dims,
                                      _ptr(self.lut), int(detail_min_count), C.byref(o), _ptr(self._ws),
                                      self._ws.numel(), _stream()),
              "sod_hough_vote_dims")
        return res


class AffineResult:
    def __init__(self, hough: HoughResult, vote_threshold: int, device):
        self.cap_valid = max(1, hough.cap_bins if vote_threshold <= 0 else
                             min(hough.cap_bins, hough.cap_votes // vote_threshold))
        self.cap_votes = hough.cap_votes
        self.counters = torch.zeros(4, dtype=torch.int32, device=device)
        self.valid_bin = torch.empty(self.cap_valid, dtype=torch.int32, device=device)
        self.params = torch.empty((self.cap_valid, 6), dtype=torch.float64, device=device)
        self.votes = torch.empty(self.cap_valid, dtype=torch.int32, device=device)
        self.status = torch.empty(self.cap_valid, dtype=torch.int32, device=device)
        self.member_keep = torch.empty(hough.cap_votes, dtype=torch.uint8, device=device)
        self._records = None

    def records(self, hough: "HoughResult"):
        if self._records is None:
            dev = self.valid_bin.device
            self._records = (torch.empty(self.cap_valid, dtype=torch.int32, device=dev),
                             torch.empty(self.cap_valid, dtype=torch.int32, device=dev),
                             torch.empty(self.cap_valid, dtype=torch.int64, device=dev),
                             torch.empty((self.cap_valid, 6), dtype=torch.float64, device=dev))
        g, c, o, m = self._records
        h, a = hough.struct(), self.struct()
        check(lib.sod_valid_bin_records(C.byref(h), C.byref(a), _ptr(g), _ptr(c), _ptr(o), _ptr(m), _stream()),
              "sod_valid_bin_records")
        return self._records

    def struct(self) -> AffineOut:
        return AffineOut(_ptr(self.counters), _ptr(self.valid_bin), _ptr(self.params), _ptr(self.votes),
                         _ptr(self.status), _ptr(self.member_keep), self.cap_valid, self.cap_votes)

    def host(self, n_votes: int) -> dict:
        c = self.counters.cpu().numpy()
        if c[1]:
            raise _capi.SodError("affine output capacity exceeded")
        nv = int(c[0])
        st = self.status[:nv].cpu().numpy()
        return dict(n_valid=nv, valid_bin=self.valid_bin[:nv].cpu().numpy(),
                    params=self.params[:nv].cpu().numpy(), votes=self.votes[:nv].cpu().numpy(),
                    live=(st & 1).astype(bool), singular=((st >> 1) & 1).astype(bool),
                    residual_edge=((st >> 2) & 1).astype(bool), passes=st >> 8,
                    n_singular=int(c[2]), n_residual_edge=int(c[3]),
                    member_keep=self.member_keep[:n_votes].cpu().numpy().astype(bool))


def affine_verify(scene: SceneArrays, match_q: torch.Tensor, match_t: torch.Tensor, hough: HoughResult,
                  vote_threshold: int = 5, affine_threshold: int = 4, factor: float = POS_FACTOR * 4,
                  result: AffineResult | None = None, factor_y: float | None = None,
                  max_passes: int = 0) -> AffineResult:
    res = result or AffineResult(hough, vote_threshold, scene.device)
    if res.cap_votes < hough.cap_votes:
        raise ValueError(f"AffineResult sized for {res.cap_votes} votes cannot take a Hough result of "
                         f"{hough.cap_votes}: build it from this HoughResult (or reserve the voter first)")
    s, h, o = scene.struct(), hough.struct(), res.struct()
    check(lib.sod_affine_verify(C.byref(s), _ptr(match_q), _ptr(match_t), C.byref(h), hough.bins,
                                int(vote_threshold), int(affine_threshold), float(factor),
                                float(factor if factor_y is None else factor_y), int(max_passes),
                                C.byref(o), _stream()), "sod_affine_verify")
    return res
```

Before: 13.26 million.

## Seed per-query pruning thresholds from DB statistics, re-sweep misses as fallback

At DB prepare time, second moments are computed over a sample of descriptors and eigendecomposed into a low-rank model of the squared-distance distribution. At match time, a predictor kernel uses that model to seed each query's threshold near the expected second-nearest distance, so the single-segment sweep can prune tiles early. Queries that end up with no valid second neighbour are compacted and re-swept exactly with a device-side plan, so results stay exact. Costs are extra kernels, extra workspace and a second sweep whose size depends on the data, and the estimate is only useful when the DB statistics match the queries.

```diff
diff --git a/include/sod.h b/include/sod.h
--- a/include/sod.h
+++ b/include/sod.h
@@ -16,6 +16,7 @@
 #define SOD_DESC_DIM 128
 #define SOD_TILE_ROWS 128
 #define SOD_CQ_TILE_INTS 260
+#define SOD_DB_STATS_FLOATS 1040
 
 typedef void* sod_stream_t;
 
@@ -41,6 +42,9 @@
 int sod_db_prepare(const uint8_t* db, int64_t n_rows, uint8_t* db_sorted, int32_t* cq, void* workspace,
                    size_t workspace_bytes, sod_stream_t stream);
 
+int sod_db_stats(const uint8_t* db, int64_t n_rows, float* stats, void* workspace, size_t workspace_bytes,
+                 sod_stream_t stream);
+
 int sod_query_prepare(const uint8_t* q, int64_t n_rows, int32_t* qn, sod_stream_t stream);
 
 size_t sod_match_workspace_bytes(int64_t n_query, int64_t n_db);
@@ -58,8 +62,8 @@
 int sod_match_top2_peer(const uint8_t* q, const int32_t* qn, int64_t n_query, const uint8_t* db_sorted,
                         const int32_t* cq, int64_t n_db, int32_t db_index_base, int64_t tile_begin,
                         int64_t tile_end, int32_t* row_thr, int32_t* const* peer_thr_host, int32_t n_peers,
-                        int64_t block_rotation, int32_t* out_idx, uint32_t* out_d2, void* workspace,
-                        size_t workspace_bytes, sod_stream_t stream);
+                        int64_t block_rotation, const float* db_stats, int32_t* out_idx, uint32_t* out_d2,
+                        void* workspace, size_t workspace_bytes, sod_stream_t stream);
 
 int sod_top2_merge(const int32_t* parts_idx, const uint32_t* parts_d2, int32_t n_parts,
                    int64_t n_query, int32_t* out_idx, uint32_t* out_d2, float* out_dist,
diff --git a/sift-based-od_b200/csrc/sod_capi.cu b/sift-based-od_b200/csrc/sod_capi.cu
--- a/sift-based-od_b200/csrc/sod_capi.cu
+++ b/sift-based-od_b200/csrc/sod_capi.cu
@@ -57,7 +57,7 @@
 
 extern "C" {
 
-int sod_version(void) { return 2000; }
+int sod_version(void) { return 3000; }
 
 const char* sod_last_error(void) { return sod::g_err; }
 
diff --git a/sift-based-od_b200/csrc/sod_match.cu b/sift-based-od_b200/csrc/sod_match.cu
--- a/sift-based-od_b200/csrc/sod_match.cu
+++ b/sift-based-od_b200/csrc/sod_match.cu
@@ -1,4 +1,7 @@
+#include <algorithm>
 #include <climits>
+#include <cmath>
+#include <vector>
 #include <cub/device/device_radix_sort.cuh>
 
 #include "sod_common.cuh"
@@ -61,6 +64,7 @@
   int n_peers;
   int unit_rot;
   int32_t* peer_thr[SOD_EXCHANGE_MAX_RANKS];
+  const int32_t* dev_plan;
 };
 
 __device__ __forceinline__ int imax3(int a, int b, int c) { return max(max(a, b), c); }
@@ -118,10 +122,13 @@
   }
 }
 
-template <bool kShare, bool kSeeded = false>
+template <bool kShare, bool kSeeded = false, bool kDevPlan = false>
 __global__ void __launch_bounds__(kThreads, 1)
 match_top2_kernel(const __grid_constant__ CUtensorMap tmap_q,
                   const __grid_constant__ CUtensorMap tmap_db, const MatchArgs a) {
+  const int nq = kDevPlan ? __ldcg(a.dev_plan) : a.nq;
+  const int n_qunits = kDevPlan ? __ldcg(a.dev_plan + 1) : a.n_qunits;
+  const int n_seg = kDevPlan ? __ldcg(a.dev_plan + 2) : a.n_seg;
   extern __shared__ uint8_t smem_raw[];
   const uint32_t raw_addr = smem_u32(smem_raw);
   const uint32_t base = (raw_addr + 1023u) & ~1023u;
@@ -172,7 +179,7 @@
   tc_fence_after();
   const uint32_t tmem_base = *tmem_ptr_smem;
 
-  const int total_units = a.n_qunits * a.n_seg;
+  const int total_units = n_qunits * n_seg;
 
   if (warp < 4) {
     if constexpr (kRegsLight < kRegsLaunch)
@@ -181,12 +188,12 @@
     if (lane == 0) {
       uint32_t step = 0, ucount = 0;
       for (int u = unit0; u < total_units; u += unit_step, ++ucount) {
-        const int seg = u / a.n_qunits;
-        int qu = u - seg * a.n_qunits + a.unit_rot;
-        if (qu >= a.n_qunits) qu -= a.n_qunits;
+        const int seg = u / n_qunits;
+        int qu = u - seg * n_qunits + a.unit_rot;
+        if (qu >= n_qunits) qu -= n_qunits;
         const int qb = qu * 2 + static_cast<int>(cta_rank);
-        const int t0 = a.tile_begin + static_cast<int>(static_cast<int64_t>(seg) * a.n_tiles / a.n_seg);
-        const int t1 = a.tile_begin + static_cast<int>(static_cast<int64_t>(seg + 1) * a.n_tiles / a.n_seg);
+        const int t0 = a.tile_begin + static_cast<int>(static_cast<int64_t>(seg) * a.n_tiles / n_seg);
+        const int t1 = a.tile_begin + static_cast<int>(static_cast<int64_t>(seg + 1) * a.n_tiles / n_seg);
         const uint32_t ab = ucount & 1u, aph = (ucount >> 1) & 1u;
         mbar_wait(bar_aempty(ab), aph ^ 1u);
         if (cta_rank == 0) mbar_arrive_expect_tx(bar_afull(ab), 2 * kQTiles * kTileBytes);
@@ -212,9 +219,9 @@
     constexpr uint32_t idesc = umma_idesc_u8(2 * kTileM, kTileN);
     uint32_t step = 0, ucount = 0;
     for (int u = unit0; u < total_units; u += unit_step, ++ucount) {
-      const int seg = u / a.n_qunits;
-      const int t0 = a.tile_begin + static_cast<int>(static_cast<int64_t>(seg) * a.n_tiles / a.n_seg);
-      const int t1 = a.tile_begin + static_cast<int>(static_cast<int64_t>(seg + 1) * a.n_tiles / a.n_seg);
+      const int seg = u / n_qunits;
+      const int t0 = a.tile_begin + static_cast<int>(static_cast<int64_t>(seg) * a.n_tiles / n_seg);
+      const int t1 = a.tile_begin + static_cast<int>(static_cast<int64_t>(seg + 1) * a.n_tiles / n_seg);
       const uint32_t ab = ucount & 1u, aph = (ucount >> 1) & 1u;
       mbar_wait(bar_afull(ab), aph);
       const uint32_t a_buf = base + kOffA + ab * (kQTiles * kTileBytes);
@@ -258,12 +265,12 @@
     asm volatile("" : "+r"(tempty_rel));
     uint32_t step = 0, ucount = 1;
     for (int u = unit0; u < total_units; u += unit_step, ++ucount) {
-      const int seg = u / a.n_qunits;
-      int qu = u - seg * a.n_qunits + a.unit_rot;
-      if (qu >= a.n_qunits) qu -= a.n_qunits;
+      const int seg = u / n_qunits;
+      int qu = u - seg * n_qunits + a.unit_rot;
+      if (qu >= n_qunits) qu -= n_qunits;
       const int qb = qu * 2 + static_cast<int>(cta_rank);
-      const int t0 = a.tile_begin + static_cast<int>(static_cast<int64_t>(seg) * a.n_tiles / a.n_seg);
-      const int t1 = a.tile_begin + static_cast<int>(static_cast<int64_t>(seg + 1) * a.n_tiles / a.n_seg);
+      const int t0 = a.tile_begin + static_cast<int>(static_cast<int64_t>(seg) * a.n_tiles / n_seg);
+      const int t1 = a.tile_begin + static_cast<int>(static_cast<int64_t>(seg + 1) * a.n_tiles / n_seg);
       const int row = qb * kBlockQ + h * kTileM + quad * 32 + lane;
       Top2 best{kNoKey64, kNoKey64, kNoKey};
       const bool thr_row = (kShare || kSeeded) && row < a.thr_rows;
@@ -307,10 +314,10 @@
           atomicMin(gthr, best.d2);
         }
       }
-      if (row < a.nq) {
+      if (row < nq) {
         const int qn = a.qn[row];
-        const int64_t o = (static_cast<int64_t>(seg) * a.nq + row) * 2;
-        SOD_DCHECK(seg < a.n_seg && (best.k1 == kNoKey64 || static_cast<int>(best.k1 & 0xFFFFFFFFll) >= a.idx_base));
+        const int64_t o = (static_cast<int64_t>(seg) * nq + row) * 2;
+        SOD_DCHECK(seg < n_seg && (best.k1 == kNoKey64 || static_cast<int>(best.k1 & 0xFFFFFFFFll) >= a.idx_base));
         const int d1 = static_cast<int>(best.k1 >> 32), d2 = static_cast<int>(best.k2 >> 32);
         a.part_d2[o + 0] = d1 != kNoKey ? static_cast<uint32_t>(d1 + qn) : 0xFFFFFFFFu;
         a.part_d2[o + 1] = d2 != kNoKey ? static_cast<uint32_t>(d2 + qn) : 0xFFFFFFFFu;
@@ -410,10 +417,124 @@
   }
 }
 
+constexpr int kStatsSample = 16384;
+constexpr int kStatsDim = SOD_DESC_DIM + 2;
+constexpr int kSpecRank = 6;
+constexpr int kSpecVecs = 2 + kSpecRank;
+constexpr int kSpecScalars = kSpecVecs * SOD_DESC_DIM;
+static_assert(kSpecScalars + 3 + kSpecRank <= SOD_DB_STATS_FLOATS && kSpecVecs == 8, "stats layout");
+constexpr double kSpecRowsBelow = 30.0;
+constexpr int64_t kSpecMinRows = 16384;
+
+__global__ void db_moments_kernel(const uint8_t* __restrict__ db, int64_t n_rows, int n_sample,
+                                  double* __restrict__ m) {
+  const int i = blockIdx.x, j = threadIdx.x;
+  if (j >= kStatsDim) return;
+  double acc = 0.0;
+  for (int r = 0; r < n_sample; ++r) {
+    const uint8_t* t = db + static_cast<int64_t>(r) * n_rows / n_sample * SOD_DESC_DIM;
+    auto elem = [&](int k) -> double {
+      if (k < SOD_DESC_DIM) return t[k];
+      if (k > SOD_DESC_DIM) return 1.0;
+      int s2 = 0;
+      for (int x = 0; x < SOD_DESC_DIM; ++x) s2 += t[x] * t[x];
+      return s2;
+    };
+    acc += elem(i) * elem(j);
+  }
+  m[i * kStatsDim + j] = acc;
+}
+
+constexpr int kPredRows = 4;
+__global__ void __launch_bounds__(256, 2) predict_thr_kernel(const uint8_t* __restrict__ q,
+                                                             const int32_t* __restrict__ qn, int64_t nq,
+                                                             int64_t thr_rows, const float* __restrict__ stats,
+                                                             float z, int32_t* __restrict__ thr,
+                                                             int32_t* __restrict__ fb_plan) {
+  const int lane = threadIdx.x & 31, part = lane & 7, half = (lane >> 3) & 1;
+  float w[4][16];
+#pragma unroll
+  for (int v = 0; v < 4; ++v)
+#pragma unroll
+    for (int k = 0; k < 16; ++k) w[v][k] = stats[(4 * half + v) * SOD_DESC_DIM + part * 16 + k];
+  float sc[3 + kSpecRank];
+#pragma unroll
+  for (int k = 0; k < 3 + kSpecRank; ++k) sc[k] = stats[kSpecScalars + k];
+  if (blockIdx.x == 0 && threadIdx.x == 0) fb_plan[0] = 0;
+  const int64_t warp0 = (static_cast<int64_t>(blockIdx.x) * blockDim.x + threadIdx.x) >> 5;
+  const int64_t stride = (static_cast<int64_t>(gridDim.x) * blockDim.x >> 5) * 2;
+  for (int64_t base = warp0 * 2 + (lane >> 4); base - (lane >> 4) < thr_rows; base += stride * kPredRows) {
+    uint4 x4[kPredRows];
+    int qr[kPredRows];
+#pragma unroll
+    for (int j = 0; j < kPredRows; ++j) {
+      const int64_t row = base + j * stride;
+      x4[j] = row < nq ? __ldg(reinterpret_cast<const uint4*>(q + row * SOD_DESC_DIM) + part) : make_uint4(0, 0, 0, 0);
+      qr[j] = row < nq ? __ldg(qn + row) : 0;
+    }
+#pragma unroll
+    for (int j = 0; j < kPredRows; ++j) {
+      const int64_t row = base + j * stride;
+      const uint32_t xw[4] = {x4[j].x, x4[j].y, x4[j].z, x4[j].w};
+      float acc[4] = {0.f, 0.f, 0.f, 0.f};
+#pragma unroll
+      for (int k = 0; k < 16; ++k) {
+        const float x = static_cast<float>((xw[k >> 2] >> (8 * (k & 3))) & 0xFFu);
+#pragma unroll
+        for (int v = 0; v < 4; ++v) acc[v] = fmaf(w[v][k], x, acc[v]);
+      }
+#pragma unroll
+      for (int v = 0; v < 4; ++v) {
+#pragma unroll
+        for (int o = 1; o < 8; o <<= 1) acc[v] += __shfl_xor_sync(0xffffffffu, acc[v], o);
+      }
+      float other[4];
+#pragma unroll
+      for (int v = 0; v < 4; ++v) other[v] = __shfl_xor_sync(0xffffffffu, acc[v], 8);
+      if ((lane & 15) == 0 && row < thr_rows) {
+        int t = kNoKey;
+        if (row < nq) {
+          const float p[kSpecRank] = {acc[2], acc[3], other[0], other[1], other[2], other[3]};
+          float quad = sc[2] * static_cast<float>(qr[j]);
+#pragma unroll
+          for (int k = 0; k < kSpecRank; ++k) quad = fmaf(sc[3 + k] * p[k], p[k], quad);
+          const float var = sc[1] - 4.f * acc[1] + 4.f * quad;
+          const float pred = sc[0] - 2.f * acc[0] - z * sqrtf(fmaxf(var, 0.f));
+          t = static_cast<int>(fminf(fmaxf(floorf(pred), -1073741824.f), static_cast<float>(kNoKey)));
+        }
+        thr[row] = t;
+      }
+    }
+  }
+}
+
+__global__ void compact_misses_kernel(const int32_t* __restrict__ out_idx, const uint8_t* __restrict__ q,
+                                      const int32_t* __restrict__ qn, int64_t nq, int32_t* __restrict__ fb_plan,
+                                      int32_t* __restrict__ row_map, uint8_t* __restrict__ q_fb,
+                                      int32_t* __restrict__ qn_fb) {
+  const int64_t row = static_cast<int64_t>(blockIdx.x) * blockDim.x + threadIdx.x;
+  const int lane = threadIdx.x & 31;
+  const bool miss = row < nq && out_idx[row * 2 + 1] < 0;
+  const unsigned m = __ballot_sync(0xffffffffu, miss);
+  if (m == 0) return;
+  int slot = 0;
+  if (lane == 0) slot = atomicAdd(fb_plan, __popc(m));
+  slot = __shfl_sync(0xffffffffu, slot, 0) + __popc(m & ((1u << lane) - 1u));
+  if (!miss) return;
+  SOD_DCHECK(slot < nq);
+  row_map[slot] = static_cast<int32_t>(row);
+  qn_fb[slot] = qn[row];
+  const uint4* src = reinterpret_cast<const uint4*>(q + row * SOD_DESC_DIM);
+  uint4* dst = reinterpret_cast<uint4*>(q_fb + static_cast<int64_t>(slot) * SOD_DESC_DIM);
+#pragma unroll
+  for (int k = 0; k < SOD_DESC_DIM / 16; ++k) dst[k] = __ldg(src + k);
+}
+
 struct PrepWs {
   uint32_t *keys_in, *keys_out;
   int32_t *vals_in, *vals_out;
   void* cub_temp;
+  double* moments;
   size_t cub_bytes, bytes;
 };
 
@@ -433,6 +554,7 @@
   cub::DeviceRadixSort::SortPairs(nullptr, w.cub_bytes, w.keys_in, w.keys_out, w.vals_in, w.vals_out,
                                   static_cast<int>(n), 0, 24);
   w.cub_temp = take(w.cub_bytes);
+  w.moments = static_cast<double*>(take(kStatsDim * kStatsDim * sizeof(double)));
   w.bytes = o;
   return w;
 }
@@ -456,15 +578,11 @@
   if (bad) atomicOr(nonint_flag, 1);
 }
 
-__global__ void top2_merge_kernel(const int32_t* __restrict__ parts_idx,
-                                  const uint32_t* __restrict__ parts_d2, int n_parts, int64_t nq,
-                                  int32_t* __restrict__ out_idx, uint32_t* __restrict__ out_d2,
-                                  float* __restrict__ out_dist, uint8_t* __restrict__ out_pass,
-                                  double ratio) {
-  const int64_t row = static_cast<int64_t>(blockIdx.x) * blockDim.x + threadIdx.x;
-  if (row >= nq) return;
-  uint32_t d1 = 0xFFFFFFFFu, d2 = 0xFFFFFFFFu;
-  int32_t i1 = -1, i2 = -1;
+__device__ __forceinline__ void merge_row(const int32_t* __restrict__ parts_idx,
+                                          const uint32_t* __restrict__ parts_d2, int n_parts, int64_t nq,
+                                          int64_t row, int32_t& i1, uint32_t& d1, int32_t& i2, uint32_t& d2) {
+  d1 = 0xFFFFFFFFu, d2 = 0xFFFFFFFFu;
+  i1 = -1, i2 = -1;
   for (int p = 0; p < n_parts; ++p) {
     const int64_t o = (static_cast<int64_t>(p) * nq + row) * 2;
     const int2 ci = *reinterpret_cast<const int2*>(parts_idx + o);
@@ -484,7 +602,32 @@
       }
     }
   }
+}
+
+__global__ void top2_merge_kernel(const int32_t* __restrict__ parts_idx,
+                                  const uint32_t* __restrict__ parts_d2, int n_parts, int64_t nq,
+                                  int32_t* __restrict__ out_idx, uint32_t* __restrict__ out_d2,
+                                  float* __restrict__ out_dist, uint8_t* __restrict__ out_pass,
+                                  double ratio) {
+  const int64_t row = static_cast<int64_t>(blockIdx.x) * blockDim.x + threadIdx.x;
+  if (row >= nq) return;
+  uint32_t d1, d2;
+  int32_t i1, i2;
+  merge_row(parts_idx, parts_d2, n_parts, nq, row, i1, d1, i2, d2);
   write_top2_row(row, i1, d1, i2, d2, out_idx, out_d2, out_dist, out_pass, ratio);
+}
+
+__global__ void top2_merge_fallback_kernel(const int32_t* __restrict__ parts_idx,
+                                           const uint32_t* __restrict__ parts_d2,
+                                           const int32_t* __restrict__ plan, const int32_t* __restrict__ row_map,
+                                           int32_t* __restrict__ out_idx, uint32_t* __restrict__ out_d2) {
+  const int64_t row = static_cast<int64_t>(blockIdx.x) * blockDim.x + threadIdx.x;
+  const int nq = plan[0];
+  if (row >= nq) return;
+  uint32_t d1, d2;
+  int32_t i1, i2;
+  merge_row(parts_idx, parts_d2, plan[2], nq, row, i1, d1, i2, d2);
+  write_top2_row(row_map[row], i1, d1, i2, d2, out_idx, out_d2, nullptr, nullptr, 0.0);
 }
 
 __global__ void top2_keys_kernel(const int32_t* __restrict__ idx, const uint32_t* __restrict__ d2, int64_t nq,
@@ -521,7 +664,7 @@
 
 constexpr int kUnitFillSteps = 6;
 
-Plan make_plan(int64_t nq, int64_t ndb, int sms) {
+__host__ __device__ Plan make_plan(int64_t nq, int64_t ndb, int sms, int64_t max_units = INT_MAX) {
   Plan p;
   p.n_tiles = static_cast<int>((ndb + kTileN - 1) / kTileN);
   p.n_qblocks = static_cast<int>((nq + kBlockQ - 1) / kBlockQ);
@@ -533,6 +676,7 @@
     int64_t best = -1;
     for (int s = 1; s <= max_seg; ++s) {
       const int64_t units = static_cast<int64_t>(p.n_qunits) * s;
+      if (s > 1 && units > max_units) break;
       const int64_t waves = (units + pairs - 1) / pairs;
       const int64_t cost = waves * ((p.n_tiles + s - 1) / s + kUnitFillSteps);
       if (best < 0 || cost < best) {
@@ -546,9 +690,61 @@
   return p;
 }
 
+__global__ void plan_fallback_kernel(int64_t n_rows_swept, int sms, int64_t max_units, int32_t* fb_plan) {
+  const Plan p = make_plan(fb_plan[0], n_rows_swept, sms, max_units);
+  fb_plan[1] = p.n_qunits;
+  fb_plan[2] = p.n_seg;
+}
+
 int make_desc_map(CUtensorMap* m, const uint8_t* ptr, int64_t n_rows, int box_rows = kTileN) {
   return make_rowmajor_map(m, CU_TENSOR_MAP_DATA_TYPE_UINT8, 1, ptr, n_rows, SOD_DESC_DIM, SOD_DESC_DIM,
                            box_rows);
+}
+
+void jacobi_eigen(double* a, int n, double* lam, double* vec) {
+  for (int i = 0; i < n; ++i)
+    for (int j = 0; j < n; ++j) vec[i * n + j] = i == j;
+  for (int sweep = 0; sweep < 50; ++sweep) {
+    double off = 0.0, diag = 0.0;
+    for (int i = 0; i < n; ++i) {
+      diag += a[i * n + i] * a[i * n + i];
+      for (int j = i + 1; j < n; ++j) off += a[i * n + j] * a[i * n + j];
+    }
+    if (off <= 1e-22 * diag) break;
+    for (int p = 0; p < n; ++p)
+      for (int q = p + 1; q < n; ++q) {
+        const double apq = a[p * n + q];
+        if (apq == 0.0) continue;
+        const double theta = (a[q * n + q] - a[p * n + p]) / (2.0 * apq);
+        const double t = (theta >= 0 ? 1.0 : -1.0) / (std::fabs(theta) + std::sqrt(theta * theta + 1.0));
+        const double c = 1.0 / std::sqrt(t * t + 1.0), s = t * c;
+        for (int k = 0; k < n; ++k) {
+          const double akp = a[k * n + p], akq = a[k * n + q];
+          a[k * n + p] = c * akp - s * akq;
+          a[k * n + q] = s * akp + c * akq;
+        }
+        for (int k = 0; k < n; ++k) {
+          const double apk = a[p * n + k], aqk = a[q * n + k];
+          a[p * n + k] = c * apk - s * aqk;
+          a[q * n + k] = s * apk + c * aqk;
+        }
+        for (int k = 0; k < n; ++k) {
+          const double vp = vec[p * n + k], vq = vec[q * n + k];
+          vec[p * n + k] = c * vp - s * vq;
+          vec[q * n + k] = s * vp + c * vq;
+        }
+      }
+  }
+  for (int i = 0; i < n; ++i) lam[i] = a[i * n + i];
+}
+
+double normal_upper_quantile(double p) {
+  double lo = 0.0, hi = 40.0;
+  for (int i = 0; i < 200; ++i) {
+    const double mid = 0.5 * (lo + hi);
+    (0.5 * std::erfc(mid / std::sqrt(2.0)) > p ? lo : hi) = mid;
+  }
+  return 0.5 * (lo + hi);
 }
 
 }
@@ -609,6 +805,57 @@
   return SOD_OK;
 }
 
+int sod_db_stats(const uint8_t* db, int64_t n_rows, float* stats, void* workspace, size_t workspace_bytes,
+                 sod_stream_t stream) {
+  SOD_CHECK_ARG(n_rows >= 0 && n_rows < (int64_t(1) << 31) - kTileN, "n_rows out of range");
+  SOD_CHECK_ARG(stats, "null pointer");
+  std::vector<float> out(SOD_DB_STATS_FLOATS, 0.f);
+  cudaStream_t st = static_cast<cudaStream_t>(stream);
+  if (n_rows > 0) {
+    SOD_CHECK_ARG(db && workspace, "null pointer");
+    SOD_CHECK_ARG((reinterpret_cast<uintptr_t>(workspace) & 255) == 0, "workspace must be 256-byte aligned");
+    PrepWs w = carve_prep_ws(workspace, n_rows);
+    SOD_CHECK_ARG(workspace_bytes >= w.bytes, "workspace too small: %zu < %zu", workspace_bytes, w.bytes);
+    const int ns = static_cast<int>(std::min<int64_t>(n_rows, kStatsSample));
+    db_moments_kernel<<<kStatsDim, 160, 0, st>>>(db, n_rows, ns, w.moments);
+    SOD_CHECK_LAUNCH("db_moments_kernel");
+    std::vector<double> m(kStatsDim * kStatsDim);
+    SOD_CHECK_CUDA(cudaMemcpyAsync(m.data(), w.moments, m.size() * sizeof(double), cudaMemcpyDeviceToHost, st));
+    SOD_CHECK_CUDA(cudaStreamSynchronize(st));
+    constexpr int D = SOD_DESC_DIM, N2 = SOD_DESC_DIM, ONE = SOD_DESC_DIM + 1;
+    auto mom = [&](int i, int j) { return m[i * kStatsDim + j] / ns; };
+    std::vector<double> sigma(D * D), lam(D), vec(D * D);
+    const double et2 = mom(N2, ONE);
+    for (int i = 0; i < D; ++i) {
+      out[i] = static_cast<float>(mom(i, ONE));
+      out[D + i] = static_cast<float>(mom(i, N2) - mom(i, ONE) * et2);
+      for (int j = 0; j < D; ++j) sigma[i * D + j] = mom(i, j) - mom(i, ONE) * mom(j, ONE);
+    }
+    jacobi_eigen(sigma.data(), D, lam.data(), vec.data());
+    std::vector<double> sorted(lam);
+    std::sort(sorted.begin(), sorted.end());
+    const double med = 0.5 * (sorted[D / 2 - 1] + sorted[D / 2]);
+    std::vector<int> order(D);
+    for (int i = 0; i < D; ++i) order[i] = i;
+    std::sort(order.begin(), order.end(),
+              [&](int x, int y) { return std::fabs(lam[x] - med) > std::fabs(lam[y] - med); });
+    double iso = 0.0;
+    for (int k = kSpecRank; k < D; ++k) iso += lam[order[k]];
+    iso /= D - kSpecRank;
+    float* sc = out.data() + kSpecScalars;
+    sc[0] = static_cast<float>(et2);
+    sc[1] = static_cast<float>(mom(N2, N2) - et2 * et2);
+    sc[2] = static_cast<float>(iso);
+    for (int k = 0; k < kSpecRank; ++k) {
+      sc[3 + k] = static_cast<float>(lam[order[k]] - iso);
+      for (int i = 0; i < D; ++i) out[(2 + k) * D + i] = static_cast<float>(vec[order[k] * D + i]);
+    }
+  }
+  SOD_CHECK_CUDA(cudaMemcpyAsync(stats, out.data(), out.size() * sizeof(float), cudaMemcpyHostToDevice, st));
+  SOD_CHECK_CUDA(cudaStreamSynchronize(st));
+  return SOD_OK;
+}
+
 int sod_query_prepare(const uint8_t* q, int64_t n_rows, int32_t* qn, sod_stream_t stream) {
   SOD_CHECK_ARG(n_rows >= 0 && n_rows < (int64_t(1) << 31) - kBlockQ, "n_rows out of range");
   if (n_rows == 0) return SOD_OK;
@@ -631,12 +878,47 @@
   return match_lists_bytes(p, n_query) + static_cast<size_t>(thr_rows(n_query)) * 4;
 }
 
+static bool speculates(const Plan& p, int64_t rows_swept) {
+  return p.n_seg == 1 && rows_swept >= kSpecMinRows;
+}
+struct SpecWs {
+  int32_t *plan, *row_map, *qn;
+  uint8_t* q;
+  uint32_t* part_d2;
+  int32_t* part_idx;
+  size_t bytes;
+};
+static SpecWs carve_spec_ws(uint8_t* base, int64_t n_query, int sms) {
+  SpecWs w;
+  size_t o = 0;
+  auto take = [&](size_t bytes) {
+    uint8_t* p = base ? base + o : nullptr;
+    o += (bytes + 255) & ~static_cast<size_t>(255);
+    return p;
+  };
+  const size_t lists = static_cast<size_t>(std::max<int64_t>(n_query, static_cast<int64_t>(sms) * 2 * kBlockQ)) * 2;
+  w.plan = reinterpret_cast<int32_t*>(take(16));
+  w.row_map = reinterpret_cast<int32_t*>(take(n_query * 4));
+  w.qn = reinterpret_cast<int32_t*>(take(n_query * 4));
+  w.q = take(n_query * SOD_DESC_DIM);
+  w.part_d2 = reinterpret_cast<uint32_t*>(take(lists * 4));
+  w.part_idx = reinterpret_cast<int32_t*>(take(lists * 4));
+  w.bytes = o;
+  return w;
+}
+static size_t match_base_bytes(const Plan& p, int64_t n_query) {
+  return (match_workspace_need(p, n_query) + 255) & ~static_cast<size_t>(255);
+}
+
 int64_t sod_row_thr_ints(int64_t n_query) { return thr_rows(n_query); }
 
 size_t sod_match_workspace_bytes(int64_t n_query, int64_t n_db) {
   if (n_query <= 0 || n_db <= 0) return 16;
-  const int sms = device_sm_count();
-  return match_workspace_need(make_plan(n_query, n_db, sms >= 2 ? sms : 148), n_query) + 16;
+  const int sms = device_sm_count() >= 2 ? device_sm_count() : 148;
+  const Plan p = make_plan(n_query, n_db, sms);
+  const int64_t rows = (n_db + kTileN - 1) / kTileN * kTileN;
+  if (!speculates(p, rows)) return match_workspace_need(p, n_query) + 16;
+  return match_base_bytes(p, n_query) + carve_spec_ws(nullptr, n_query, sms).bytes + 16;
 }
 
 int sod_match_top2(const uint8_t* q, const int32_t* qn, int64_t n_query, const uint8_t* db_sorted,
@@ -651,14 +933,14 @@
                          int64_t tile_end, int32_t* row_thr, int32_t* out_idx, uint32_t* out_d2,
                          void* workspace, size_t workspace_bytes, sod_stream_t stream) {
   return sod_match_top2_peer(q, qn, n_query, db_sorted, cq, n_db, db_index_base, tile_begin, tile_end, row_thr, nullptr, 0,
-                             0, out_idx, out_d2, workspace, workspace_bytes, stream);
+                             0, nullptr, out_idx, out_d2, workspace, workspace_bytes, stream);
 }
 
 int sod_match_top2_peer(const uint8_t* q, const int32_t* qn, int64_t n_query, const uint8_t* db_sorted,
                         const int32_t* cq, int64_t n_db, int32_t db_index_base, int64_t tile_begin,
                         int64_t tile_end, int32_t* row_thr, int32_t* const* peer_thr_host, int32_t n_peers,
-                        int64_t block_rotation, int32_t* out_idx, uint32_t* out_d2, void* workspace,
-                        size_t workspace_bytes, sod_stream_t stream) {
+                        int64_t block_rotation, const float* db_stats, int32_t* out_idx, uint32_t* out_d2,
+                        void* workspace, size_t workspace_bytes, sod_stream_t stream) {
   SOD_CHECK_ARG(n_peers >= 0 && n_peers <= SOD_EXCHANGE_MAX_RANKS && (n_peers == 0 || (peer_thr_host && row_thr)),
                 "bad peer threshold table");
   SOD_CHECK_ARG(block_rotation >= 0, "negative block rotation");
@@ -693,8 +975,12 @@
     set_error("sod_match_top2: the matcher runs on CTA pairs and needs at least 2 SMs, the device has %d", sms);
     return SOD_ERR_UNSUPPORTED;
   }
-  const Plan p = make_plan(n_query, (tile_end - tile_begin) * kTileN, sms);
-  const size_t need = match_workspace_need(p, n_query);
+  const int64_t rows_swept = (tile_end - tile_begin) * kTileN;
+  const Plan p = make_plan(n_query, rows_swept, sms);
+  const bool spec = !row_thr && db_stats && speculates(p, rows_swept);
+  const SpecWs sw = carve_spec_ws(spec ? static_cast<uint8_t*>(workspace) + match_base_bytes(p, n_query) : nullptr,
+                                  n_query, sms);
+  const size_t need = spec ? match_base_bytes(p, n_query) + sw.bytes : match_workspace_need(p, n_query);
   SOD_CHECK_ARG(workspace_bytes >= need, "workspace too small: %zu < %zu", workspace_bytes, need);
 
   CUtensorMap map_q, map_db;
@@ -709,9 +995,18 @@
   a.part_d2 = static_cast<uint32_t*>(workspace);
   a.part_idx = reinterpret_cast<int32_t*>(a.part_d2 + static_cast<size_t>(p.n_seg) * n_query * 2);
   a.row_thr = row_thr;
-  if (!row_thr && p.n_seg > 1) {
-    a.row_thr = reinterpret_cast<int32_t*>(static_cast<uint8_t*>(workspace) + match_lists_bytes(p, n_query));
-    SOD_CHECK_CUDA(cudaMemsetAsync(a.row_thr, 0x7F, static_cast<size_t>(thr_rows(n_query)) * 4, st));
+  int32_t* const own_thr = reinterpret_cast<int32_t*>(static_cast<uint8_t*>(workspace) + match_lists_bytes(p, n_query));
+  const size_t own_thr_bytes = static_cast<size_t>(thr_rows(n_query)) * 4;
+  if (spec) {
+    a.row_thr = own_thr;
+    const double z = normal_upper_quantile(kSpecRowsBelow / static_cast<double>(rows_swept));
+    predict_thr_kernel<<<static_cast<unsigned>(std::min<int64_t>((thr_rows(n_query) + 16 * kPredRows - 1) /
+                                                                  (16 * kPredRows), 2 * sms)), 256, 0,
+                         st>>>(q, qn, n_query, thr_rows(n_query), db_stats, static_cast<float>(z), own_thr, sw.plan);
+    SOD_CHECK_LAUNCH("predict_thr_kernel");
+  } else if (!row_thr && p.n_seg > 1) {
+    a.row_thr = own_thr;
+    SOD_CHECK_CUDA(cudaMemsetAsync(a.row_thr, 0x7F, own_thr_bytes, st));
   }
   a.nq = static_cast<int>(n_query);
   a.thr_rows = static_cast<int>(thr_rows(n_query));
@@ -720,20 +1015,19 @@
   a.n_qunits = p.n_qunits;
   a.n_seg = p.n_seg;
   a.idx_base = db_index_base;
+  a.dev_plan = nullptr;
   const bool peer_mode = n_peers > 0 && row_thr && p.n_seg == 1;
   a.n_peers = peer_mode ? n_peers : 0;
   a.unit_rot = peer_mode ? static_cast<int>((block_rotation / (2 * kBlockQ / kAbiBlockQ)) % p.n_qunits) : 0;
   for (int i = 0; i < SOD_EXCHANGE_MAX_RANKS; ++i) a.peer_thr[i] = (peer_mode && i < n_peers) ? peer_thr_host[i] : nullptr;
   for (int i = 0; i < a.n_peers; ++i) SOD_CHECK_ARG(a.peer_thr[i], "null threshold array of rank %d", i);
 
-  const bool seeded = row_thr && p.n_seg == 1, share = a.row_thr && !seeded;
+  const bool seeded = (row_thr || spec) && p.n_seg == 1, share = a.row_thr && !seeded;
   auto* kernel = seeded ? match_top2_kernel<false, true>
                         : share ? match_top2_kernel<true, false> : match_top2_kernel<false, false>;
-  SOD_CHECK_CUDA(cudaFuncSetAttribute(kernel, cudaFuncAttributeMaxDynamicSharedMemorySize, kSmemBytes));
-  {
-    StageScope timed(SOD_STAGE_MATCH, st);
+  auto launch = [&](decltype(kernel) k, int grid, const CUtensorMap& mq, const MatchArgs& args) {
     cudaLaunchConfig_t cfg = {};
-    cfg.gridDim = dim3(static_cast<unsigned>(p.grid));
+    cfg.gridDim = dim3(static_cast<unsigned>(grid));
     cfg.blockDim = dim3(kThreads);
     cfg.dynamicSmemBytes = static_cast<size_t>(kSmemBytes);
     cfg.stream = st;
@@ -744,12 +1038,41 @@
     attr[0].val.clusterDim.z = 1;
     cfg.attrs = attr;
     cfg.numAttrs = 1;
-    SOD_CHECK_CUDA(cudaLaunchKernelEx(&cfg, kernel, map_q, map_db, a));
+    return cudaLaunchKernelEx(&cfg, k, mq, map_db, args);
+  };
+  SOD_CHECK_CUDA(cudaFuncSetAttribute(kernel, cudaFuncAttributeMaxDynamicSharedMemorySize, kSmemBytes));
+  {
+    StageScope timed(SOD_STAGE_MATCH, st);
+    SOD_CHECK_CUDA(launch(kernel, p.grid, map_q, a));
   }
   SOD_CHECK_LAUNCH("match_top2_kernel");
   top2_merge_kernel<<<mblocks, mthreads, 0, st>>>(a.part_idx, a.part_d2, p.n_seg, n_query,
                                                   out_idx, out_d2, nullptr, nullptr, 0.0);
   SOD_CHECK_LAUNCH("top2_merge_kernel");
+  if (!spec) return SOD_OK;
+
+  compact_misses_kernel<<<static_cast<unsigned>((n_query + 255) / 256), 256, 0, st>>>(
+      out_idx, q, qn, n_query, sw.plan, sw.row_map, sw.q, sw.qn);
+  SOD_CHECK_LAUNCH("compact_misses_kernel");
+  plan_fallback_kernel<<<1, 1, 0, st>>>(rows_swept, sms, sms, sw.plan);
+  SOD_CHECK_LAUNCH("plan_fallback_kernel");
+  SOD_CHECK_CUDA(cudaMemsetAsync(own_thr, 0x7F, own_thr_bytes, st));
+  CUtensorMap map_fb;
+  rc = make_desc_map(&map_fb, sw.q, n_query);
+  if (rc != SOD_OK) return rc;
+  MatchArgs f = a;
+  f.qn = sw.qn;
+  f.part_d2 = sw.part_d2;
+  f.part_idx = sw.part_idx;
+  f.row_thr = own_thr;
+  f.dev_plan = sw.plan;
+  auto* fb_kernel = match_top2_kernel<true, false, true>;
+  SOD_CHECK_CUDA(cudaFuncSetAttribute(fb_kernel, cudaFuncAttributeMaxDynamicSharedMemorySize, kSmemBytes));
+  SOD_CHECK_CUDA(launch(fb_kernel, sms / 2 * 2, map_fb, f));
+  SOD_CHECK_LAUNCH("match_top2_kernel (re-sweep)");
+  top2_merge_fallback_kernel<<<mblocks, mthreads, 0, st>>>(sw.part_idx, sw.part_d2, sw.plan, sw.row_map, out_idx,
+                                                           out_d2);
+  SOD_CHECK_LAUNCH("top2_merge_fallback_kernel");
   return SOD_OK;
 }
 
diff --git a/sift-based-od_b200/sod_b200/_capi.py b/sift-based-od_b200/sod_b200/_capi.py
--- a/sift-based-od_b200/sod_b200/_capi.py
+++ b/sift-based-od_b200/sod_b200/_capi.py
@@ -9,6 +9,7 @@
 SOD_OK = 0
 DESC_DIM = 128
 TILE_ROWS = 128
+DB_STATS_FLOATS = 1040
 
 
 class SodError(RuntimeError):
@@ -86,13 +87,14 @@
     "sod_pack_u8_from_f32": (C.c_int, [_p, _i64, _p, _p, _p]),
     "sod_db_prepare_workspace_bytes": (C.c_size_t, [_i64]),
     "sod_db_prepare": (C.c_int, [_p, _i64, _p, _p, _p, C.c_size_t, _p]),
+    "sod_db_stats": (C.c_int, [_p, _i64, _p, _p, C.c_size_t, _p]),
     "sod_query_prepare": (C.c_int, [_p, _i64, _p, _p]),
     "sod_match_workspace_bytes": (C.c_size_t, [_i64, _i64]),
     "sod_match_top2": (C.c_int, [_p, _p, _i64, _p, _p, _i64, _i32, _p, _p, _p, C.c_size_t, _p]),
     "sod_row_thr_ints": (_i64, [_i64]),
     "sod_match_top2_range": (C.c_int, [_p, _p, _i64, _p, _p, _i64, _i32, _i64, _i64, _p, _p, _p, _p, C.c_size_t, _p]),
     "sod_match_top2_peer": (C.c_int, [_p, _p, _i64, _p, _p, _i64, _i32, _i64, _i64, _p, _p, _i32, _i64, _p, _p, _p,
-                                      C.c_size_t, _p]),
+                                      _p, C.c_size_t, _p]),
     "sod_top2_merge": (C.c_int, [_p, _p, _i32, _i64, _p, _p, _p, _p, C.c_double, _p]),
     "sod_top2_keys": (C.c_int, [_p, _p, _i64, _i64, _p, _p]),
     "sod_top2_merge_keys": (C.c_int, [_p, _i32, _i64, _p, _p]),
diff --git a/sift-based-od_b200/sod_b200/engine.py b/sift-based-od_b200/sod_b200/engine.py
--- a/sift-based-od_b200/sod_b200/engine.py
+++ b/sift-based-od_b200/sod_b200/engine.py
@@ -57,6 +57,7 @@
     n_rows: int
     cq: torch.Tensor
     index_base: int
+    stats: torch.Tensor
 
     @property
     def n(self) -> int:
@@ -73,7 +74,9 @@
     ws = torch.empty(int(lib.sod_db_prepare_workspace_bytes(n)), dtype=torch.uint8, device=dev)
     check(lib.sod_db_prepare(_ptr(des_u8), n, _ptr(des_sorted), _ptr(cq), _ptr(ws), ws.numel(),
                              _stream()), "sod_db_prepare")
-    return DescriptorShard(des_sorted, n, cq, int(index_base))
+    stats = torch.empty(_capi.DB_STATS_FLOATS, dtype=torch.float32, device=dev)
+    check(lib.sod_db_stats(_ptr(des_u8), n, _ptr(stats), _ptr(ws), ws.numel(), _stream()), "sod_db_stats")
+    return DescriptorShard(des_sorted, n, cq, int(index_base), stats)
 
 
 class Matcher:
@@ -118,7 +121,8 @@
         n_peers = 0 if peer_table is None else len(peer_table)
         check(lib.sod_match_top2_peer(_ptr(q_u8), _ptr(qn), nq, _ptr(s.des), _ptr(s.cq), s.n, s.index_base, t0, t1,
                                       _ptr(row_thr), None if peer_table is None else C.cast(peer_table, C.c_void_p),
-                                      n_peers, int(block_rotation), _ptr(idx), _ptr(d2), _ptr(ws), ws.numel(),
+                                      n_peers, int(block_rotation), _ptr(s.stats), _ptr(idx), _ptr(d2), _ptr(ws),
+                                      ws.numel(),
                                       _stream()), "sod_match_top2_peer")
         if self.events is not None:
             e1.record()
```

Result: faster. 13.48 million, median of 6 (+1.7%).
